# Aazmp/vp8oclenc

Measured on AMD Instinct MI355X. Metric: macroblocks/sec inter-frame (ME+DCT+loopfilter), 1080p, higher is better.
Workload: dtype u8/int32

## Files before the change

vp8oclenc_amd/csrc/kernels_mb.hip:

```cpp
#include <stdlib.h>
#include <string.h>

#include "vp8hip_dev.h"

namespace vp8 {


struct TDiv { uint32_t M8; bool one; };
struct Recip24 { uint32_t m8[512]; };
static constexpr Recip24 make_recip24() {
    Recip24 t{};
    for (uint32_t q = 0; q < 512; ++q) t.m8[q] = q < 2 ? 0u : (((1u << 24) / q + 1u) << 8);
    return t;
}
static __device__ __constant__ const Recip24 k_recip24 = make_recip24();
__device__ __forceinline__ TDiv tdiv_make(int q) { return TDiv{k_recip24.m8[q & 511], q == 1}; }
__device__ __forceinline__ int tdiv(int x, const TDiv &d) {
    const int s = x >> 31;
    const uint32_t n = (uint32_t)((x ^ s) - s);
    const uint32_t r = d.one ? n : __umulhi(n, d.M8);
    return ((int)r ^ s) - s;
}

constexpr uint32_t pk8t(int a, int b, int c, int d) {
    return (uint32_t)(a & 255) | ((uint32_t)(b & 255) << 8) | ((uint32_t)(c & 255) << 16) | ((uint32_t)(d & 255) << 24);
}
#define P6(f0, f1, f2, f3, f4, f5)                                                                          \
    {pk8t(f0, f1, f2, f3), pk8t(f4, f5, 0, 0), pk8t(0, f0, f1, f2), pk8t(f3, f4, f5, 0), pk8t(0, 0, f0, f1),  \
     pk8t(f2, f3, f4, f5), pk8t(0, 0, 0, f0),  pk8t(f1, f2, f3, f4), pk8t(f5, 0, 0, 0),  0, 0, 0}
static __device__ __constant__ const uint32_t K_P6[8][12] = {
    P6(0, 0, 0, 0, 0, 0),       P6(0, -6, 123, 12, -1, 0), P6(2, -11, 108, 36, -8, 1), P6(0, -9, 93, 50, -6, 0),
    P6(3, -16, 77, 77, -16, 3), P6(0, -6, 50, 93, -9, 0),  P6(1, -8, 36, 108, -11, 2), P6(0, -1, 12, 123, -6, 0)};
constexpr int KB6 = 128 * 128 + 64;
__device__ __forceinline__ int d4k(uint32_t a, uint32_t b, int c) { return __builtin_amdgcn_sdot4((int)a, (int)b, c, true); }
__device__ __forceinline__ int d4(uint32_t a, uint32_t b, int c) { return __builtin_amdgcn_sdot4((int)a, (int)b, c, false); }
__device__ __forceinline__ void six_tap4(uint32_t w0, uint32_t w1, uint32_t w2, const uint32_t t[9], int s[4]) {
    s[0] = d4(w1, t[1], d4k(w0, t[0], KB6));
    s[1] = d4(w1, t[3], d4k(w0, t[2], KB6));
    s[2] = d4(w1, t[5], d4k(w0, t[4], KB6));
    s[3] = d4(w2, t[8], d4(w1, t[7], d4k(w0, t[6], KB6)));
}
__device__ __forceinline__ uint32_t pack_sat4(const int s[4]) {
    const uint32_t lo = __builtin_amdgcn_ashr_pk_u8_i32(s[0], s[1], 7), hi = __builtin_amdgcn_ashr_pk_u8_i32(s[2], s[3], 7);
    return __builtin_amdgcn_perm(hi, lo, 0x05040100u);
}
template <bool CONFORMANT>
__device__ __forceinline__ void predict4x4(const Plane &rf, int ix, int iy, int fx, int fy, uint32_t out[4]) {
    uint32_t tx[9], ty[9];
#pragma unroll
    for (int i = 0; i < 9; ++i) { tx[i] = K_P6[fx][i]; ty[i] = K_P6[fy][i]; }
    uint32_t Hb[9];
#pragma unroll
    for (int L = 0; L < 9; ++L) {
        const uint8_t *p = rf.p + (ptrdiff_t)(iy - 2 + L) * rf.stride + (ix - 2);
        const uint32_t w0 = ld_u32(p) ^ 0x80808080u, w1 = ld_u32(p + 4) ^ 0x80808080u, w2 = ld_u32(p + 8) ^ 0x80808080u;
        int sm[4];
        six_tap4(w0, w1, w2, tx, sm);
        uint32_t h;
        if (L < 6 || CONFORMANT) {
            h = pack_sat4(sm);
        } else {
            h = 0;
#pragma unroll
            for (int c = 0; c < 4; ++c) h |= (uint32_t)(div128(sm[c]) & 0xff) << (8 * c);
        }
        h ^= 0x80808080u;
        Hb[L] = fx == 0 ? __builtin_amdgcn_alignbyte(w1, w0, 2) : h;
    }
    uint32_t ca[4], cb[4], oc[4];
    transpose4x4(Hb, ca);
    transpose4x4(Hb + 4, cb);
#pragma unroll
    for (int c = 0; c < 4; ++c) {
        int sm[4];
        six_tap4(ca[c], cb[c], Hb[8] >> (8 * c), ty, sm);
        const uint32_t v = pack_sat4(sm);
        oc[c] = fy == 0 ? (__builtin_amdgcn_alignbyte(cb[c], ca[c], 2) ^ 0x80808080u) : v;
    }
    transpose4x4(oc, out);
}

__device__ __forceinline__ void fdct4x4(const int in[16], int out[16]) {
    int L[16];
#pragma unroll
    for (int c = 0; c < 4; ++c) {
        const int r0 = in[c], r1 = in[4 + c], r2 = in[8 + c], r3 = in[12 + c];
        const int a1 = (r0 + r3) * 8, d1 = (r0 - r3) * 8, b1 = (r1 + r2) * 8, c1 = (r1 - r2) * 8;
        L[c] = a1 + b1;
        L[8 + c] = a1 - b1;
        const uint32_t xy = pk16(c1, d1);
        L[4 + c] = dot2(xy, K_ROT_A, 14500) >> 12;
        L[12 + c] = dot2(xy, K_ROT_B, 7500) >> 12;
    }
#pragma unroll
    for (int i = 0; i < 4; ++i) {
        const int e0 = L[4 * i], e1 = L[4 * i + 1], e2 = L[4 * i + 2], e3 = L[4 * i + 3];
        const int a1 = e0 + e3, d1 = e0 - e3, b1 = e1 + e2, c1 = e1 - e2;
        out[4 * i] = (a1 + b1 + 7) >> 4;
        out[4 * i + 2] = (a1 - b1 + 7) >> 4;
        const uint32_t xy = pk16(c1, d1);
        out[4 * i + 1] = (dot2(xy, K_ROT_A, 12000) >> 16) + (d1 != 0);
        out[4 * i + 3] = dot2(xy, K_ROT_B, 51000) >> 16;
    }
}

__device__ __forceinline__ void idct4x4(int L[16]) {
    int T[16];
#pragma unroll
    for (int c = 0; c < 4; ++c) {
        const int i0 = L[c], i1 = L[4 + c], i2 = L[8 + c], i3 = L[12 + c];
        const int a1 = i0 + i2, b1 = i0 - i2;
        const int c1 = (__mul24(i1, 35468) >> 16) - (i3 + (__mul24(i3, 20091) >> 16));
        const int d1 = (i1 + (__mul24(i1, 20091) >> 16)) + (__mul24(i3, 35468) >> 16);
        T[c] = a1 + d1;
        T[12 + c] = a1 - d1;
        T[4 + c] = b1 + c1;
        T[8 + c] = b1 - c1;
    }
#pragma unroll
    for (int r = 0; r < 4; ++r) {
        const int i0 = T[4 * r], i1 = T[4 * r + 1], i2 = T[4 * r + 2], i3 = T[4 * r + 3];
        const int a1 = i0 + i2, b1 = i0 - i2;
        const int c1 = (__mul24(i1, 35468) >> 16) - (i3 + (__mul24(i3, 20091) >> 16));
        const int d1 = (i1 + (__mul24(i1, 20091) >> 16)) + (__mul24(i3, 35468) >> 16);
        L[4 * r] = (a1 + d1 + 4) >> 3;
        L[4 * r + 3] = (a1 - d1 + 4) >> 3;
        L[4 * r + 1] = (b1 + c1 + 4) >> 3;
        L[4 * r + 2] = (b1 - c1 + 4) >> 3;
    }
}

__device__ __forceinline__ int had4(int v0, int v1, int v2, int v3, int i) {
    const int s1 = i >= 2 ? -1 : 1, s2 = (i == 1 || i == 2) ? -1 : 1, s3 = (i & 1) ? -1 : 1;
    return v0 + __mul24(s1, v1) + __mul24(s2, v2) + __mul24(s3, v3);
}
__device__ __forceinline__ int wht_roundtrip_lane(int x, int lane, int dc_q, int ac_q, const TDiv &ddc, const TDiv &dac, int &q) {
    const int L = lane & 15, r = L >> 2, c = L & 3;
    const int base = (int)(threadIdx.x & 32u) * 4;
    const int col = base + 4 * c, row = base + 4 * (L & 12);
    auto gather_col = [&](int v, int i) { return had4(__builtin_amdgcn_ds_bpermute(col, v), __builtin_amdgcn_ds_bpermute(col + 16, v),
                                                      __builtin_amdgcn_ds_bpermute(col + 32, v), __builtin_amdgcn_ds_bpermute(col + 48, v), i); };
    auto gather_row = [&](int v, int i) { return had4(__builtin_amdgcn_ds_bpermute(row, v), __builtin_amdgcn_ds_bpermute(row + 4, v),
                                                      __builtin_amdgcn_ds_bpermute(row + 8, v), __builtin_amdgcn_ds_bpermute(row + 12, v), i); };
    int o = gather_row(gather_col(x, r), c);
    o += (o > 0);
    o >>= 1;
    q = tdiv(o, L == 0 ? ddc : dac);
    const int xq = __mul24(q, L == 0 ? dc_q : ac_q);
    return (gather_col(gather_row(xq, c), r) + 3) >> 3;
}

__device__ __forceinline__ constexpr int inv_zigzag(int k) {
    constexpr int t[16] = {0, 1, 5, 6, 2, 4, 7, 12, 3, 8, 11, 13, 9, 10, 14, 15};
    return t[k];
}
__device__ __forceinline__ int inv_zigzag_rt(int k) { return (int)((0xfea9db83c7426510ull >> (4 * k)) & 15); }
__device__ __forceinline__ void store_zigzag(int16_t *dst, const int L[16]) {
    int z[16];
#pragma unroll
    for (int k = 0; k < 16; ++k) z[inv_zigzag(k)] = L[k];
    uint32_t w[8];
#pragma unroll
    for (int k = 0; k < 8; ++k) w[k] = (uint32_t)(uint16_t)z[2 * k] | ((uint32_t)(uint16_t)z[2 * k + 1] << 16);
    uint4 *d4 = reinterpret_cast<uint4 *>(dst);
    d4[0] = make_uint4(w[0], w[1], w[2], w[3]);
    d4[1] = make_uint4(w[4], w[5], w[6], w[7]);
}

struct MBPlanes { uint8_t *y, *u, *v; };
struct MBArgs {
    MBPlanes cur, ref0, ref1, ref2, recon;
    int ystride, cstride, yw, yh, cw, ch;
    int32_t *o_parts, *o_ref, *o_seg, *o_nz, *o_mask;
    int16_t *o_vec, *o_coeffs;
    float *o_ssim;
    int32_t *o_flag;
    const SegData *sd;
    const int32_t *bdiff0, *bdiff1, *bdiff2;
    const int16_t *vnet0, *vnet1, *vnet2;
    float ssim_target;
    int mbw, mbs;
    int use_golden, use_altref;
};

struct MBTile { uint8_t cur[384]; uint8_t rec[384]; float fa[384]; float fb[384]; };

__device__ __forceinline__ void tile_sums(const uint32_t *t32, int lane, int &sy, int &sc) {
    sy = (int)__builtin_amdgcn_sad_u8(t32[lane], 0u, __builtin_amdgcn_sad_u8(t32[lane + 32], 0u, 0u));
    sc = (int)__builtin_amdgcn_sad_u8(t32[64 + lane], 0u, 0u);
#pragma unroll
    for (int m = 16; m >= 1; m >>= 1) sy += __shfl_xor(sy, m, 32);
#pragma unroll
    for (int m = 8; m >= 1; m >>= 1) sc += __shfl_xor(sc, m, 32);
}
__device__ __forceinline__ float chain(const float *p, int n4) {
    float acc = 0.0f;
    for (int q = 0; q < n4; q += 4) {
        const float4 v = *reinterpret_cast<const float4 *>(p + q);
        acc = q == 0 ? v.x : __fadd_rn(v.x, acc);
        acc = __fadd_rn(v.y, acc);
        acc = __fadd_rn(v.z, acc);
        acc = __fadd_rn(v.w, acc);
    }
    return acc;
}
__device__ __forceinline__ float sum4(float acc, int lane) {
    const float s0 = __shfl(acc, (lane & ~3) + 0, 32), s1 = __shfl(acc, (lane & ~3) + 1, 32);
    const float s2 = __shfl(acc, (lane & ~3) + 2, 32), s3 = __shfl(acc, (lane & ~3) + 3, 32);
    return __fadd_rn(__fadd_rn(__fadd_rn(s0, s1), s2), s3);
}

template <bool CONFORMANT>
__device__ __forceinline__ void mb_body(const MBArgs &a, MBTile *s_t) {
    const int g = threadIdx.x >> 5, lane = threadIdx.x & 31;
    const int mb_raw = xcd_band(blockIdx.x, gridDim.x) * 8 + g;
    const bool live = mb_raw < a.mbs;
    const int mb = live ? mb_raw : a.mbs - 1;
    const int mbx = mb % a.mbw, mby = mb / a.mbw;
    const int32_t *SD = a.sd->v;

    const bool blk = lane < 24;
    const int plane = lane < 16 ? 0 : (lane < 20 ? 1 : 2);
    const int bi = lane < 16 ? lane : (lane - 16) & 3;
    const int bw = plane == 0 ? 4 : 2;
    const int bx = blk ? bi % bw : 0, by = blk ? bi / bw : 0;
    const int msz = plane == 0 ? 16 : 8;
    const int posx = mbx * msz + bx * 4, posy = mby * msz + by * 4;
    const int b8w = a.mbw * 2;
    const int cell0 = (mby * 2) * b8w + mbx * 2;
    const int cidx[4] = {cell0, cell0 + 1, cell0 + b8w, cell0 + b8w + 1};
    int diff1 = a.bdiff0[cidx[0]] + a.bdiff0[cidx[1]] + a.bdiff0[cidx[2]] + a.bdiff0[cidx[3]];
    int diff2 = 0x7fffffff;
    if (a.use_altref == 1)
        diff2 = a.bdiff2[cidx[0]] + a.bdiff2[cidx[1]] + a.bdiff2[cidx[2]] + a.bdiff2[cidx[3]];
    int ref = diff1 <= diff2 ? 0 : 2;
    diff1 = diff1 <= diff2 ? diff1 : diff2;
    diff2 = 0x7fffffff;
    if (a.use_golden == 1)
        diff2 = a.bdiff1[cidx[0]] + a.bdiff1[cidx[1]] + a.bdiff1[cidx[2]] + a.bdiff1[cidx[3]];
    ref = diff1 <= diff2 ? ref : 1;
    const uint32_t *vnet = reinterpret_cast<const uint32_t *>(ref == 0 ? a.vnet0 : (ref == 1 ? a.vnet1 : a.vnet2));
    uint32_t mbv[4];
#pragma unroll
    for (int k = 0; k < 4; ++k) mbv[k] = vnet[cidx[k]];
    const int parts = (mbv[1] == mbv[0] && mbv[2] == mbv[0] && mbv[3] == mbv[0]) ? 0 : 1;
    if (lane == 0 && live) {
        a.o_ref[mb] = ref;
        a.o_parts[mb] = parts;
        *reinterpret_cast<uint4 *>(a.o_vec + 8 * mb) = make_uint4(mbv[0], mbv[1], mbv[2], mbv[3]);
    }
    uint8_t *const rpy = ref == 0 ? a.ref0.y : (ref == 1 ? a.ref1.y : a.ref2.y);
    uint8_t *const rpu = ref == 0 ? a.ref0.u : (ref == 1 ? a.ref1.u : a.ref2.u);
    uint8_t *const rpv = ref == 0 ? a.ref0.v : (ref == 1 ? a.ref1.v : a.ref2.v);
    const int pstride = plane == 0 ? a.ystride : a.cstride, pw = plane == 0 ? a.yw : a.cw, ph = plane == 0 ? a.yh : a.ch;
    const Plane cp{plane == 0 ? a.cur.y : (plane == 1 ? a.cur.u : a.cur.v), pstride, pw, ph};
    const Plane rc{plane == 0 ? a.recon.y : (plane == 1 ? a.recon.u : a.recon.v), pstride, pw, ph};
    const Plane rp{plane == 0 ? rpy : (plane == 1 ? rpu : rpv), pstride, pw, ph};
    const int tile_off = plane == 0 ? 0 : (plane == 1 ? 256 : 320);

    uint32_t predw[4] = {0, 0, 0, 0};
    if (blk) {
        const int quad = plane == 0 ? (by >> 1) * 2 + (bx >> 1) : by * 2 + bx;
        const uint32_t vv = quad == 0 ? mbv[0] : (quad == 1 ? mbv[1] : (quad == 2 ? mbv[2] : mbv[3]));
        const int vx = (int16_t)(vv & 0xffffu), vy = (int16_t)(vv >> 16);
        const int gsh = plane == 0 ? 2 : 3, gm = plane == 0 ? 3 : 7;
        const int fxp = posx * (gm + 1) + vx, fyp = posy * (gm + 1) + vy;
        const int dx = (fxp & gm) * (plane == 0 ? 2 : 1), dy = (fyp & gm) * (plane == 0 ? 2 : 1);
        const int ix = iclamp(fxp >> gsh, 2 - EXT, rp.w + EXT - 7), iy = iclamp(fyp >> gsh, 2 - EXT, rp.h + EXT - 7);
        predict4x4<CONFORMANT>(rp, ix, iy, dx, dy, predw);
#pragma unroll
        for (int r = 0; r < 4; ++r) {
            const uint32_t cw = *reinterpret_cast<const uint32_t *>(cp.p + (ptrdiff_t)(posy + r) * cp.stride + posx);
            *reinterpret_cast<uint32_t *>(&s_t[g].cur[tile_off + (by * 4 + r) * msz + bx * 4]) = cw;
        }
    }
    const int sp = (lane >> 2) < 3 ? (lane >> 2) : 2, comp = lane & 3;
    const int n4 = sp == 0 ? 64 : 16;
    const int chain_off = (sp == 0 ? 0 : (sp == 1 ? 256 : 320)) + comp * n4;
    const float area = sp == 0 ? 256.0f : 64.0f;
    const uint32_t *cur32 = reinterpret_cast<const uint32_t *>(s_t[g].cur);
    const uint32_t *rec32 = reinterpret_cast<const uint32_t *>(s_t[g].rec);
    const int coff = (lane < 16 ? 256 : 320) + (lane & 15);
    float *fa = s_t[g].fa, *fb = s_t[g].fb;
    float M1y, M1c, M1, D1;
    {
        int sy, sc;
        tile_sums(cur32, lane, sy, sc);
        M1y = __fdiv_rn((float)sy, 256.0f);
        M1c = __fdiv_rn((float)sc, 64.0f);
        const float mu = __shfl(M1c, 0, 32), mv = __shfl(M1c, 16, 32);
        M1 = sp == 0 ? M1y : (sp == 1 ? mu : mv);
#pragma unroll
        for (int h = 0; h < 3; ++h) {
            const uint32_t w = cur32[h < 2 ? lane + 32 * h : 64 + lane];
            const float m = h < 2 ? M1y : M1c;
            const int off = h < 2 ? lane + 32 * h : coff, cs = h < 2 ? 64 : 16;
#pragma unroll
            for (int k = 0; k < 4; ++k) {
                const float t = __fsub_rn((float)byte_of(w, k), m);
                fa[off + k * cs] = __fmul_rn(t, t);
            }
        }
        D1 = __fdiv_rn(sum4(chain(fa + chain_off, n4), lane), area);
    }

    float ssim = -2.0f;
    int seg_final = a.o_seg[mb];
    int nz_blk = 0;
    bool any_pass = false;

    for (int seg = 3; seg >= 0; --seg) {
        if (ssim > a.ssim_target) break;
        {
        any_pass = true;
        seg_final = seg;
        const int i = SD[seg * SD_INTS + SD_Y_AC_I];
        int dc_q, ac_q;
        if (plane == 0) {
            ac_q = k_ac_q[i];
            dc_q = parts == 0 ? 1 : k_dc_q[qi(SD[SD_Y_DC_IDELTA] + i)];
        } else {
            dc_q = imin(k_dc_q[qi(SD[SD_UV_DC_IDELTA] + i)], 132);
            ac_q = k_ac_q[qi(SD[SD_UV_AC_IDELTA] + i)];
        }
        int coef[16];
#pragma unroll
        for (int k = 0; k < 16; ++k) coef[k] = 0;
        if (blk) {
            int res[16];
#pragma unroll
            for (int r = 0; r < 4; ++r) {
                const uint32_t cw = *reinterpret_cast<const uint32_t *>(&s_t[g].cur[tile_off + (by * 4 + r) * msz + bx * 4]);
#pragma unroll
                for (int c = 0; c < 4; ++c) res[4 * r + c] = byte_of(cw, c) - byte_of(predw[r], c);
            }
            fdct4x4(res, coef);
            const TDiv ddc = tdiv_make(dc_q), dac = tdiv_make(ac_q);
            coef[0] = tdiv(coef[0], ddc);
#pragma unroll
            for (int k = 1; k < 16; ++k) coef[k] = tdiv(coef[k], dac);
        }
        nz_blk = 0;
        if (parts == 0) {
            const int y2dc = k_dc_q[qi(SD[SD_Y2_DC_IDELTA] + i)] * 2;
            const int y2ac = imax(31 * k_ac_q[qi(SD[SD_Y2_AC_IDELTA] + i)] / 20, 8);
            int q24 = 0;
            const int nd = wht_roundtrip_lane((int16_t)coef[0], lane, y2dc, y2ac, tdiv_make(y2dc), tdiv_make(y2ac), q24);
            if (lane < 16) {
                coef[0] = (int16_t)nd;
                if (live) a.o_coeffs[((size_t)mb * 25 + 24) * 16 + inv_zigzag_rt(lane)] = (int16_t)q24;
                nz_blk += iabs((int16_t)q24);
            }
        }
        if (blk) {
            if (live) store_zigzag(a.o_coeffs + ((size_t)mb * 25 + lane) * 16, coef);
#pragma unroll
            for (int k = 1; k < 16; ++k) nz_blk += iabs((int16_t)coef[k]);
            if (plane != 0 || parts != 0) nz_blk += iabs((int16_t)coef[0]);
            int L[16];
            L[0] = __mul24((int16_t)coef[0], dc_q);
#pragma unroll
            for (int k = 1; k < 16; ++k) L[k] = __mul24((int16_t)coef[k], ac_q);
            idct4x4(L);
#pragma unroll
            for (int r = 0; r < 4; ++r) {
                uint32_t w = 0;
#pragma unroll
                for (int c = 0; c < 4; ++c) w |= (uint32_t)sat8(L[4 * r + c] + byte_of(predw[r], c)) << (8 * c);
                *reinterpret_cast<uint32_t *>(&s_t[g].rec[tile_off + (by * 4 + r) * msz + bx * 4]) = w;
                if (live) *reinterpret_cast<uint32_t *>(rc.p + (ptrdiff_t)(posy + r) * rc.stride + posx) = w;
            }
        }
        }
        {
        float M2, D, C;
        {
            int sy, sc;
            tile_sums(rec32, lane, sy, sc);
            const float M2y = __fdiv_rn((float)sy, 256.0f), M2c = __fdiv_rn((float)sc, 64.0f);
            const float mu = __shfl(M2c, 0, 32), mv = __shfl(M2c, 16, 32);
            M2 = sp == 0 ? M2y : (sp == 1 ? mu : mv);
#pragma unroll
            for (int h = 0; h < 3; ++h) {
                const int di = h < 2 ? lane + 32 * h : 64 + lane;
                const uint32_t wc = cur32[di], wr = rec32[di];
                const float m1 = h < 2 ? M1y : M1c, m2 = h < 2 ? M2y : M2c;
                const int off = h < 2 ? lane + 32 * h : coff, cs = h < 2 ? 64 : 16;
#pragma unroll
                for (int k = 0; k < 4; ++k) {
                    const float t1 = __fsub_rn((float)byte_of(wc, k), m1);
                    const float t2 = __fsub_rn((float)byte_of(wr, k), m2);
                    fa[off + k * cs] = __fmul_rn(t2, t2);
                    fb[off + k * cs] = __fmul_rn(t1, t2);
                }
            }
            D = __fadd_rn(D1, __fdiv_rn(sum4(chain(fa + chain_off, n4), lane), area));
            C = __fdiv_rn(sum4(chain(fb + chain_off, n4), lane), area);
        }
        const float k1 = 0.01f * 0.01f * 255 * 255, k2 = 0.03f * 0.03f * 255 * 255;
        const float num = __fmul_rn(__fadd_rn(__fmul_rn(M1, __fmul_rn(M2, 2.0f)), k1), __fadd_rn(__fmul_rn(C, 2.0f), k2));
        const float den = __fmul_rn(__fadd_rn(__fmul_rn(M1, M1), __fadd_rn(__fmul_rn(M2, M2), k1)), __fadd_rn(D, k2));
        float metric = __fdiv_rn(num, den);
        float dm = __fsub_rn(M1, M2);
        dm = dm < 0 ? -dm : dm;
        dm = dm > 4 ? __fmul_rn(0.02f, dm) : 0.0f;
        metric = __fsub_rn(metric, dm);
        const float m1 = __shfl(metric, 0, 32), m2 = __shfl(metric, 4, 32), m3 = __shfl(metric, 8, 32);
        ssim = __fdiv_rn(__fadd_rn(__fadd_rn(m1, m2), m3), 3.0f);
        }
    }

    int nz = any_pass ? nz_blk : 0;
#pragma unroll
    for (int m = 16; m >= 1; m >>= 1) nz += __shfl_xor(nz, m, 32);
    if (lane == 0 && live) {
        if (any_pass) {
            a.o_seg[mb] = seg_final;
            a.o_nz[mb] = nz;
            a.o_mask[mb] = (parts != 0 || nz > 0) ? -1 : 0;
        }
        a.o_ssim[mb] = ssim;
        if (ssim < a.ssim_target) *a.o_flag = 1;
    }
}

struct MBShare {
    float M1[8][4], M2[8][4], D1[8][4], metric[8][4];
    int nzc[8];
    int any[2];
};
struct MBTileP { MBTile t; uint32_t skew[4]; };
template <int CTRL>
__device__ __forceinline__ int dpp_i(int v) { return __builtin_amdgcn_update_dpp(0, v, CTRL, 0xf, 0xf, false); }
template <int CTRL>
__device__ __forceinline__ float dpp_f(float v) { return __builtin_bit_cast(float, dpp_i<CTRL>(__builtin_bit_cast(int, v))); }
__device__ __forceinline__ int quad_sum(int v) {
    v += dpp_i<0xb1>(v);
    return v + dpp_i<0x4e>(v);
}
__device__ __forceinline__ int half_row_sum(int v) { v = quad_sum(v); return v + dpp_i<0x141>(v); }
__device__ __forceinline__ int row_sum(int v) { v = half_row_sum(v); return v + dpp_i<0x140>(v); }
__device__ __forceinline__ float sum4_quad(float acc) {
    return __fadd_rn(__fadd_rn(__fadd_rn(dpp_f<0x00>(acc), dpp_f<0x55>(acc)), dpp_f<0xaa>(acc)), dpp_f<0xff>(acc));
}
template <int N4>
__device__ __forceinline__ float chain_n(const float *p) {
    float acc = 0.0f;
#pragma unroll 4
    for (int q = 0; q < N4; q += 4) {
        const float4 v = *reinterpret_cast<const float4 *>(p + q);
        acc = q == 0 ? v.x : __fadd_rn(v.x, acc);
        acc = __fadd_rn(v.y, acc);
        acc = __fadd_rn(v.z, acc);
        acc = __fadd_rn(v.w, acc);
    }
    return acc;
}
__device__ __forceinline__ int wht_roundtrip_row(int x, int L, int base_bytes, int dc_q, int ac_q, const TDiv &ddc, const TDiv &dac, int &q) {
    const int r = L >> 2, c = L & 3;
    const int col = base_bytes + 4 * c, row = base_bytes + 4 * (L & 12);
    auto gather_col = [&](int v, int i) { return had4(__builtin_amdgcn_ds_bpermute(col, v), __builtin_amdgcn_ds_bpermute(col + 16, v),
                                                      __builtin_amdgcn_ds_bpermute(col + 32, v), __builtin_amdgcn_ds_bpermute(col + 48, v), i); };
    auto gather_row = [&](int v, int i) { return had4(__builtin_amdgcn_ds_bpermute(row, v), __builtin_amdgcn_ds_bpermute(row + 4, v),
                                                      __builtin_amdgcn_ds_bpermute(row + 8, v), __builtin_amdgcn_ds_bpermute(row + 12, v), i); };
    int o = gather_row(gather_col(x, r), c);
    o += (o > 0);
    o >>= 1;
    q = tdiv(o, L == 0 ? ddc : dac);
    const int xq = __mul24(q, L == 0 ? dc_q : ac_q);
    return (gather_col(gather_row(xq, c), r) + 3) >> 3;
}

template <bool CONFORMANT>
__device__ __forceinline__ void mb_body_packed(const MBArgs &a, MBTileP *s_t, MBShare *s_x) {
    const int w = __builtin_amdgcn_readfirstlane((int)(threadIdx.x >> 6)), wl = threadIdx.x & 63;
    const bool luma = w < 2;
    const int g = luma ? w * 4 + (wl >> 4) : wl >> 3;
    const int plane = luma ? 0 : 1 + ((wl >> 2) & 1);
    const int bi = luma ? wl & 15 : wl & 3;
    const int blkidx = luma ? bi : 12 + 4 * plane + bi;
    const int mb_raw = xcd_band(blockIdx.x, gridDim.x) * 8 + g;
    const bool live = mb_raw < a.mbs;
    const int mb = live ? mb_raw : a.mbs - 1;
    const int mbx = mb % a.mbw, mby = mb / a.mbw;
    const int32_t *SD = a.sd->v;
    const int bw = luma ? 4 : 2;
    const int bx = bi % bw, by = bi / bw;
    const int msz = luma ? 16 : 8;
    const int posx = mbx * msz + bx * 4, posy = mby * msz + by * 4;
    if (threadIdx.x == 0) s_x->any[0] = s_x->any[1] = 0;
    const int b8w = a.mbw * 2;
    const int cell0 = (mby * 2) * b8w + mbx * 2;
    const int cidx[4] = {cell0, cell0 + 1, cell0 + b8w, cell0 + b8w + 1};
    int diff1 = a.bdiff0[cidx[0]] + a.bdiff0[cidx[1]] + a.bdiff0[cidx[2]] + a.bdiff0[cidx[3]];
    int diff2 = 0x7fffffff;
    if (a.use_altref == 1)
        diff2 = a.bdiff2[cidx[0]] + a.bdiff2[cidx[1]] + a.bdiff2[cidx[2]] + a.bdiff2[cidx[3]];
    int ref = diff1 <= diff2 ? 0 : 2;
    diff1 = diff1 <= diff2 ? diff1 : diff2;
    diff2 = 0x7fffffff;
    if (a.use_golden == 1)
        diff2 = a.bdiff1[cidx[0]] + a.bdiff1[cidx[1]] + a.bdiff1[cidx[2]] + a.bdiff1[cidx[3]];
    ref = diff1 <= diff2 ? ref : 1;
    const uint32_t *vnet = reinterpret_cast<const uint32_t *>(ref == 0 ? a.vnet0 : (ref == 1 ? a.vnet1 : a.vnet2));
    uint32_t mbv[4];
#pragma unroll
    for (int k = 0; k < 4; ++k) mbv[k] = vnet[cidx[k]];
    const int parts = (mbv[1] == mbv[0] && mbv[2] == mbv[0] && mbv[3] == mbv[0]) ? 0 : 1;
    const bool head = luma && bi == 0;
    if (head && live) {
        a.o_ref[mb] = ref;
        a.o_parts[mb] = parts;
        *reinterpret_cast<uint4 *>(a.o_vec + 8 * mb) = make_uint4(mbv[0], mbv[1], mbv[2], mbv[3]);
    }
    uint8_t *const rpy = ref == 0 ? a.ref0.y : (ref == 1 ? a.ref1.y : a.ref2.y);
    uint8_t *const rpu = ref == 0 ? a.ref0.u : (ref == 1 ? a.ref1.u : a.ref2.u);
    uint8_t *const rpv = ref == 0 ? a.ref0.v : (ref == 1 ? a.ref1.v : a.ref2.v);
    const int pstride = luma ? a.ystride : a.cstride, pw = luma ? a.yw : a.cw, ph = luma ? a.yh : a.ch;
    const Plane cp{plane == 0 ? a.cur.y : (plane == 1 ? a.cur.u : a.cur.v), pstride, pw, ph};
    const Plane rc{plane == 0 ? a.recon.y : (plane == 1 ? a.recon.u : a.recon.v), pstride, pw, ph};
    const Plane rp{plane == 0 ? rpy : (plane == 1 ? rpu : rpv), pstride, pw, ph};
    const int tile_off = plane == 0 ? 0 : (plane == 1 ? 256 : 320);
    MBTile &T = s_t[g].t;

    uint32_t predw[4];
    {
        const int quad = luma ? (by >> 1) * 2 + (bx >> 1) : by * 2 + bx;
        const uint32_t vv = quad == 0 ? mbv[0] : (quad == 1 ? mbv[1] : (quad == 2 ? mbv[2] : mbv[3]));
        const int vx = (int16_t)(vv & 0xffffu), vy = (int16_t)(vv >> 16);
        const int gsh = luma ? 2 : 3, gm = luma ? 3 : 7;
        const int fxp = posx * (gm + 1) + vx, fyp = posy * (gm + 1) + vy;
        const int dx = (fxp & gm) * (luma ? 2 : 1), dy = (fyp & gm) * (luma ? 2 : 1);
        const int ix = iclamp(fxp >> gsh, 2 - EXT, rp.w + EXT - 7), iy = iclamp(fyp >> gsh, 2 - EXT, rp.h + EXT - 7);
        predict4x4<CONFORMANT>(rp, ix, iy, dx, dy, predw);
#pragma unroll
        for (int r = 0; r < 4; ++r) {
            const uint32_t cw = *reinterpret_cast<const uint32_t *>(cp.p + (ptrdiff_t)(posy + r) * cp.stride + posx);
            *reinterpret_cast<uint32_t *>(&T.cur[tile_off + (by * 4 + r) * msz + bx * 4]) = cw;
        }
    }
    const uint32_t *cur32 = reinterpret_cast<const uint32_t *>(T.cur) + (tile_off >> 2);
    const uint32_t *rec32 = reinterpret_cast<const uint32_t *>(T.rec) + (tile_off >> 2);
    const int dstep = luma ? 16 : 4, cs = luma ? 64 : 16;
    const float area = luma ? 256.0f : 64.0f;
    float *fa = T.fa + tile_off + bi, *fb = T.fb + tile_off + bi;
    auto plane_sum = [&](const uint32_t *t32) {
        uint32_t s = 0;
#pragma unroll
        for (int h = 0; h < 4; ++h) s = __builtin_amdgcn_sad_u8(t32[bi + dstep * h], 0u, s);
        return luma ? row_sum((int)s) : quad_sum((int)s);
    };
    const float M1 = __fdiv_rn((float)plane_sum(cur32), area);
#pragma unroll
    for (int h = 0; h < 4; ++h) {
        const uint32_t wd = cur32[bi + dstep * h];
#pragma unroll
        for (int k = 0; k < 4; ++k) {
            const float t = __fsub_rn((float)byte_of(wd, k), M1);
            fa[dstep * h + k * cs] = __fmul_rn(t, t);
        }
    }
    if (bi == 0) s_x->M1[g][plane] = M1;
    __syncthreads();
    if (w == 0) {
        if (wl < 32) {
            const int m = wl >> 2, comp = wl & 3;
            const float s = sum4_quad(chain_n<64>(s_t[m].t.fa + comp * 64));
            if (comp == 0) s_x->D1[m][0] = __fdiv_rn(s, 256.0f);
        }
    } else if (w == 1) {
        const int m = wl >> 3, p = 1 + ((wl >> 2) & 1), comp = wl & 3;
        const float s = sum4_quad(chain_n<16>(s_t[m].t.fa + (p == 1 ? 256 : 320) + comp * 16));
        if (comp == 0) s_x->D1[m][p] = __fdiv_rn(s, 64.0f);
    }
    __syncthreads();

    float ssim = -2.0f;
    int seg_final = a.o_seg[mb];
    int nz_y = 0, nz_c = 0;
    bool any_pass = false;
    for (int seg = 3, round = 0; seg >= 0; --seg, ++round) {
        const bool act = !(ssim > a.ssim_target);
        if (act) {
            any_pass = true;
            seg_final = seg;
            const int i = SD[seg * SD_INTS + SD_Y_AC_I];
            int dc_q, ac_q;
            if (luma) {
                ac_q = k_ac_q[i];
                dc_q = parts == 0 ? 1 : k_dc_q[qi(SD[SD_Y_DC_IDELTA] + i)];
            } else {
                dc_q = imin(k_dc_q[qi(SD[SD_UV_DC_IDELTA] + i)], 132);
                ac_q = k_ac_q[qi(SD[SD_UV_AC_IDELTA] + i)];
            }
            int coef[16];
            {
                int res[16];
#pragma unroll
                for (int r = 0; r < 4; ++r) {
                    const uint32_t cw = *reinterpret_cast<const uint32_t *>(&T.cur[tile_off + (by * 4 + r) * msz + bx * 4]);
#pragma unroll
                    for (int c = 0; c < 4; ++c) res[4 * r + c] = byte_of(cw, c) - byte_of(predw[r], c);
                }
                fdct4x4(res, coef);
                const TDiv ddc = tdiv_make(dc_q), dac = tdiv_make(ac_q);
                coef[0] = tdiv(coef[0], ddc);
#pragma unroll
                for (int k = 1; k < 16; ++k) coef[k] = tdiv(coef[k], dac);
            }
            int nz_blk = 0;
            if (luma && parts == 0) {
                const int y2dc = k_dc_q[qi(SD[SD_Y2_DC_IDELTA] + i)] * 2;
                const int y2ac = imax(31 * k_ac_q[qi(SD[SD_Y2_AC_IDELTA] + i)] / 20, 8);
                int q24 = 0;
                const int nd = wht_roundtrip_row((int16_t)coef[0], bi, (wl & 48) * 4, y2dc, y2ac, tdiv_make(y2dc), tdiv_make(y2ac), q24);
                coef[0] = (int16_t)nd;
                if (live) a.o_coeffs[((size_t)mb * 25 + 24) * 16 + inv_zigzag_rt(bi)] = (int16_t)q24;
                nz_blk += iabs((int16_t)q24);
            }
            {
                if (live) store_zigzag(a.o_coeffs + ((size_t)mb * 25 + blkidx) * 16, coef);
#pragma unroll
                for (int k = 1; k < 16; ++k) nz_blk += iabs((int16_t)coef[k]);
                if (!luma || parts != 0) nz_blk += iabs((int16_t)coef[0]);
                int L[16];
                L[0] = __mul24((int16_t)coef[0], dc_q);
#pragma unroll
                for (int k = 1; k < 16; ++k) L[k] = __mul24((int16_t)coef[k], ac_q);
                idct4x4(L);
#pragma unroll
                for (int r = 0; r < 4; ++r) {
                    uint32_t wd = 0;
#pragma unroll
                    for (int c = 0; c < 4; ++c) wd |= (uint32_t)sat8(L[4 * r + c] + byte_of(predw[r], c)) << (8 * c);
                    *reinterpret_cast<uint32_t *>(&T.rec[tile_off + (by * 4 + r) * msz + bx * 4]) = wd;
                    if (live) *reinterpret_cast<uint32_t *>(rc.p + (ptrdiff_t)(posy + r) * rc.stride + posx) = wd;
                }
            }
            if (luma) nz_y = row_sum(nz_blk);
            else {
                const int n = half_row_sum(nz_blk);
                if ((wl & 7) == 0) s_x->nzc[g] = n;
            }
            const float M2 = __fdiv_rn((float)plane_sum(rec32), area);
#pragma unroll
            for (int h = 0; h < 4; ++h) {
                const uint32_t wc = cur32[bi + dstep * h], wr = rec32[bi + dstep * h];
#pragma unroll
                for (int k = 0; k < 4; ++k) {
                    const float t1 = __fsub_rn((float)byte_of(wc, k), M1);
                    const float t2 = __fsub_rn((float)byte_of(wr, k), M2);
                    fa[dstep * h + k * cs] = __fmul_rn(t2, t2);
                    fb[dstep * h + k * cs] = __fmul_rn(t1, t2);
                }
            }
            if (bi == 0) {
                s_x->M2[g][plane] = M2;
                s_x->any[round & 1] = 1;
            }
        }
        __syncthreads();
        if (!s_x->any[round & 1]) break;
        if (threadIdx.x == 0) s_x->any[(round + 1) & 1] = 0;
        {
            const int comp = wl & 3;
            const int m = w == 0 ? (wl >> 2) & 7 : (w - 1) * 4 + ((wl >> 3) & 3);
            const int p = w == 0 ? 0 : 1 + ((wl >> 2) & 1);
            const float *src = (wl < 32 ? s_t[m].t.fa : s_t[m].t.fb) + (p == 0 ? 0 : (p == 1 ? 256 : 320)) + comp * (w == 0 ? 64 : 16);
            const float acc = w == 0 ? chain_n<64>(src) : chain_n<16>(src);
            const float s = __fdiv_rn(sum4_quad(acc), w == 0 ? 256.0f : 64.0f);
            const float C = __shfl_xor(s, 32, 64);
            const float D = __fadd_rn(s_x->D1[m][p], s);
            const float m1v = s_x->M1[m][p], m2v = s_x->M2[m][p];
            const float k1 = 0.01f * 0.01f * 255 * 255, k2 = 0.03f * 0.03f * 255 * 255;
            const float num = __fmul_rn(__fadd_rn(__fmul_rn(m1v, __fmul_rn(m2v, 2.0f)), k1), __fadd_rn(__fmul_rn(C, 2.0f), k2));
            const float den = __fmul_rn(__fadd_rn(__fmul_rn(m1v, m1v), __fadd_rn(__fmul_rn(m2v, m2v), k1)), __fadd_rn(D, k2));
            float metric = __fdiv_rn(num, den);
            float dm = __fsub_rn(m1v, m2v);
            dm = dm < 0 ? -dm : dm;
            dm = dm > 4 ? __fmul_rn(0.02f, dm) : 0.0f;
            metric = __fsub_rn(metric, dm);
            if (wl < 32 && comp == 0) s_x->metric[m][p] = metric;
        }
        if (act && luma) nz_c = s_x->nzc[g];
        __syncthreads();
        const float4 mt = *reinterpret_cast<const float4 *>(s_x->metric[g]);
        ssim = __fdiv_rn(__fadd_rn(__fadd_rn(mt.x, mt.y), mt.z), 3.0f);
    }

    if (head && live) {
        if (any_pass) {
            const int nz = nz_y + nz_c;
            a.o_seg[mb] = seg_final;
            a.o_nz[mb] = nz;
            a.o_mask[mb] = (parts != 0 || nz > 0) ? -1 : 0;
        }
        a.o_ssim[mb] = ssim;
        if (ssim < a.ssim_target) *a.o_flag = 1;
    }
}

__global__ __launch_bounds__(256, 2) void k_mb_b(BatchOf<MBArgs> b) {
    __shared__ __attribute__((aligned(16))) MBTile s_t[8];
    mb_body<false>(b.item[blockIdx.z], s_t);
}
__global__ __launch_bounds__(256, 2) void k_mb_b_conformant(BatchOf<MBArgs> b) {
    __shared__ __attribute__((aligned(16))) MBTile s_t[8];
    mb_body<true>(b.item[blockIdx.z], s_t);
}

__global__ __launch_bounds__(192, 2) void k_mb_p(BatchOf<MBArgs> b) {
    __shared__ __attribute__((aligned(16))) MBTileP s_t[8];
    __shared__ __attribute__((aligned(16))) MBShare s_x;
    mb_body_packed<false>(b.item[blockIdx.z], s_t, &s_x);
}
__global__ __launch_bounds__(192, 2) void k_mb_p_conformant(BatchOf<MBArgs> b) {
    __shared__ __attribute__((aligned(16))) MBTileP s_t[8];
    __shared__ __attribute__((aligned(16))) MBShare s_x;
    mb_body_packed<true>(b.item[blockIdx.z], s_t, &s_x);
}
static bool mb_packed() {
    static const bool on = [] { const char *v = getenv("VP8HIP_MB_PACKED"); return !(v && v[0] == '0'); }();
    return on;
}

static MBArgs mb_args(const CodingItem &it, float ssim_target, int mbw, int mbh) {
    const Frame &cur = *it.cur, &recon = *it.recon;
    const RefSet &refs = it.refs;
    const NetSet &nets = *it.nets;
    const MBOut &o = *it.out;
    MBArgs a;
    auto planes = [](const Frame &f) { return MBPlanes{f.Y[0].p, f.U.p, f.V.p}; };
    a.cur = planes(cur);
    a.ref0 = planes(refs.ref[0]); a.ref1 = planes(refs.ref[1]); a.ref2 = planes(refs.ref[2]);
    a.recon = planes(recon);
    a.ystride = cur.Y[0].stride; a.yw = cur.Y[0].w; a.yh = cur.Y[0].h;
    a.cstride = cur.U.stride; a.cw = cur.U.w; a.ch = cur.U.h;
    a.o_parts = o.parts; a.o_ref = o.ref; a.o_seg = o.seg; a.o_nz = o.nz; a.o_mask = o.mask;
    a.o_vec = o.vec; a.o_coeffs = o.coeffs; a.o_ssim = o.ssim; a.o_flag = o.flags;
    a.sd = it.sd;
    a.bdiff0 = nets.bdiff[0]; a.bdiff1 = nets.bdiff[1]; a.bdiff2 = nets.bdiff[2];
    a.vnet0 = nets.net[0][0]; a.vnet1 = nets.net[1][0]; a.vnet2 = nets.net[2][0];
    a.ssim_target = ssim_target;
    a.mbw = mbw;
    a.mbs = mbw * mbh;
    a.use_golden = refs.use[1];
    a.use_altref = refs.use[2];
    return a;
}
static bool mb_skip() {
    static const bool skip = experiment_skip("mb");
    return skip;
}

void launch_mb_batch(hipStream_t s, const CodingItem *items, int n, float ssim_target, int mbw, int mbh, bool conformant) {
    static_assert(sizeof(BatchOf<MBArgs>) <= 4096, "the batch travels in the kernel arguments");
    BatchOf<MBArgs> b;
    b.n = n;
    for (int i = 0; i < n; ++i) b.item[i] = mb_args(items[i], ssim_target, mbw, mbh);
    if (mb_skip()) return;
    const dim3 grid((b.item[0].mbs + 7) / 8, 1, n);
    if (mb_packed()) {
        if (conformant) VP8_LAUNCH(k_mb_p_conformant, grid, dim3(192), 0, s, b);
        else VP8_LAUNCH(k_mb_p, grid, dim3(192), 0, s, b);
        return;
    }
    if (conformant) VP8_LAUNCH(k_mb_b_conformant, grid, dim3(256), 0, s, b);
    else VP8_LAUNCH(k_mb_b, grid, dim3(256), 0, s, b);
}

__global__ __launch_bounds__(256) void k_filter_mask(MBOut o, const SegData *sd, int mbs) {
    const int lane = threadIdx.x & 31;
    const int mb_raw = blockIdx.x * 8 + (threadIdx.x >> 5);
    const bool live = mb_raw < mbs;
    const int mb = live ? mb_raw : mbs - 1;
    const int parts = o.parts[mb];
    int nz = 0;
    if (lane < 25) {
        const int16_t *c = o.coeffs + ((size_t)mb * 25 + lane) * 16;
        int s = 0;
#pragma unroll
        for (int k = 1; k < 16; ++k) s += iabs(c[k]);
        if (lane < 16) nz = s + (parts != 0 ? iabs(c[0]) : 0);
        else if (lane < 24) nz = s + iabs(c[0]);
        else nz = parts == 0 ? s + iabs(c[0]) : 0;
    }
#pragma unroll
    for (int m = 16; m >= 1; m >>= 1) nz += __shfl_xor(nz, m, 32);
    if (lane == 0 && live) {
        o.nz[mb] = nz;
        o.mask[mb] = (parts != 0 || nz > 0) ? -1 : 0;
    }
}

void launch_filter_mask(hipStream_t s, const MBOut &o, const SegData *d_sd, int mbs) {
    hipLaunchKernelGGL(k_filter_mask, dim3((mbs + 7) / 8), dim3(256), 0, s, o, d_sd, mbs);
}

}
```

vp8oclenc_amd/csrc/kernels_me.hip:

```cpp
#include <stdlib.h>
#include <string.h>

#include "vp8hip_dev.h"
#include "s1_pre_layout.h"
#include "s1_fill_layout.h"

namespace vp8 {

struct BorderItem { Plane y, u, v; };
static_assert(EXT == 8, "border_row stores a margin as one eight-byte word");
__device__ __forceinline__ void border_row(const Plane &pl, int row, int lane) {
    if (row >= pl.h + EXT) return;
    uint8_t *dst = pl.p + (ptrdiff_t)row * pl.stride;
    const uint8_t *src = pl.p + (ptrdiff_t)iclamp(row, 0, pl.h - 1) * pl.stride;
    if (row < 0 || row >= pl.h)
        for (int x = lane * 8; x < pl.w; x += 512) *reinterpret_cast<uint2 *>(dst + x) = *reinterpret_cast<const uint2 *>(src + x);
    if (lane < 2) {
        const uint32_t s4 = (uint32_t)src[lane ? pl.w - 1 : 0] * 0x01010101u;
        *reinterpret_cast<uint2 *>(dst + (lane ? pl.w : -EXT)) = make_uint2(s4, s4);
    }
}
__device__ __forceinline__ void border_body(const BorderItem &a) {
    border_row(blockIdx.y == 0 ? a.y : (blockIdx.y == 1 ? a.u : a.v), (int)blockIdx.x - EXT, threadIdx.x);
}

__global__ __launch_bounds__(64) void k_border(BorderItem a) { border_body(a); }

void launch_border(hipStream_t s, const Frame &f) {
    dim3 grid(f.Y[0].h + 2 * EXT, 3);
    VP8_LAUNCH(k_border, grid, dim3(64), 0, s, BorderItem{f.Y[0], f.U, f.V});
}

struct PyrArgs { Frame f[2 * MAX_BATCH]; uint32_t border_mask; };
static int border_jobs(const Frame &f) { return (f.Y[0].h + 2 * EXT) + 2 * (f.U.h + 2 * EXT); }

__global__ __launch_bounds__(256) void k_pyramid(PyrArgs a) {
    __shared__ uint8_t s2[16][16];
    __shared__ uint8_t s3[8][8];
    const Frame &f = a.f[blockIdx.z];
    const int t = threadIdx.x, tx = t & 15, ty = t >> 4;
    const Plane &P0 = f.Y[0];
    const int tiles_y = (P0.h + 63) / 64;
    const int tile = xcd_band((int)blockIdx.y * (int)gridDim.x + (int)blockIdx.x, tiles_y * (int)gridDim.x);
    const int bx = tile % (int)gridDim.x, by = tile / (int)gridDim.x;
    if ((int)blockIdx.y >= tiles_y) {
        if (!((a.border_mask >> blockIdx.z) & 1)) return;
        int job = (((int)blockIdx.y - tiles_y) * (int)gridDim.x + (int)blockIdx.x) * 4 + (t >> 6);
        const int ny = P0.h + 2 * EXT, nc = f.U.h + 2 * EXT;
        if (job < ny) border_row(P0, job - EXT, t & 63);
        else if (job < ny + nc) border_row(f.U, job - ny - EXT, t & 63);
        else if (job < ny + 2 * nc) border_row(f.V, job - ny - nc - EXT, t & 63);
        return;
    }
    const int sx = imin(bx * 64 + 4 * tx, P0.w - 4), sy0 = by * 64 + 4 * ty;
    uint32_t r[4];
#pragma unroll
    for (int k = 0; k < 4; ++k)
        r[k] = *reinterpret_cast<const uint32_t *>(P0.p + (ptrdiff_t)imin(sy0 + k, P0.h - 1) * P0.stride + sx);
    int l1[2][2];
#pragma unroll
    for (int j = 0; j < 2; ++j)
#pragma unroll
        for (int i = 0; i < 2; ++i)
            l1[j][i] = (byte_of(r[2 * j], 2 * i) + byte_of(r[2 * j], 2 * i + 1) + byte_of(r[2 * j + 1], 2 * i) +
                        byte_of(r[2 * j + 1], 2 * i + 1) + 2) >> 2;
    const Plane &P1 = f.Y[1];
    const int x1 = bx * 32 + 2 * tx, y1 = by * 32 + 2 * ty;
    if (x1 < P1.w) {
#pragma unroll
        for (int j = 0; j < 2; ++j)
            if (y1 + j < P1.h)
                *reinterpret_cast<uint16_t *>(P1.p + (ptrdiff_t)(y1 + j) * P1.stride + x1) = (uint16_t)(l1[j][0] | (l1[j][1] << 8));
    }
    const int l2 = (l1[0][0] + l1[0][1] + l1[1][0] + l1[1][1] + 2) >> 2;
    const Plane &P2 = f.Y[2];
    const int x2 = bx * 16 + tx, y2 = by * 16 + ty;
    if (x2 < P2.w && y2 < P2.h) P2.p[(ptrdiff_t)y2 * P2.stride + x2] = (uint8_t)l2;
    s2[ty][tx] = (uint8_t)l2;
    __syncthreads();
    if (t < 64) {
        const int ux = t & 7, uy = t >> 3;
        const int l3 = (s2[2 * uy][2 * ux] + s2[2 * uy][2 * ux + 1] + s2[2 * uy + 1][2 * ux] + s2[2 * uy + 1][2 * ux + 1] + 2) >> 2;
        const Plane &P3 = f.Y[3];
        const int x3 = bx * 8 + ux, y3 = by * 8 + uy;
        if (x3 < P3.w && y3 < P3.h) P3.p[(ptrdiff_t)y3 * P3.stride + x3] = (uint8_t)l3;
        s3[uy][ux] = (uint8_t)l3;
    }
    __syncthreads();
    if (t < 16) {
        const int ux = t & 3, uy = t >> 2;
        const int l4 = (s3[2 * uy][2 * ux] + s3[2 * uy][2 * ux + 1] + s3[2 * uy + 1][2 * ux] + s3[2 * uy + 1][2 * ux + 1] + 2) >> 2;
        const Plane &P4 = f.Y[4];
        const int x4 = bx * 4 + ux, y4 = by * 4 + uy;
        if (x4 < P4.w && y4 < P4.h) P4.p[(ptrdiff_t)y4 * P4.stride + x4] = (uint8_t)l4;
    }
}

static dim3 pyramid_grid(const Frame &f, int nframes, uint32_t border_mask) {
    const int gx = (f.Y[0].w + 63) / 64, gy = (f.Y[0].h + 63) / 64;
    const int extra = border_mask ? ((border_jobs(f) + 3) / 4 + gx - 1) / gx : 0;
    return dim3(gx, gy + extra, nframes);
}
void launch_pyramid(hipStream_t s, const Frame *a, const Frame *b, uint32_t border_mask) {
    PyrArgs p;
    p.f[0] = *a;
    p.f[1] = b ? *b : *a;
    p.border_mask = border_mask;
    VP8_LAUNCH(k_pyramid, pyramid_grid(*a, b ? 2 : 1, border_mask), dim3(256), 0, s, p);
}
void launch_pyramid_batch(hipStream_t s, const Frame *const *f, int nframes, uint32_t border_mask) {
    if (nframes <= 0) return;
    PyrArgs p;
    for (int i = 0; i < nframes; ++i) p.f[i] = *f[i];
    p.border_mask = border_mask;
    VP8_LAUNCH(k_pyramid, pyramid_grid(*f[0], nframes, border_mask), dim3(256), 0, s, p);
}

struct PackItem { Plane py, pu, pv; const uint8_t *sy, *su, *sv; int sw, sh, ssy, ssc; };
__device__ __forceinline__ void pack_body(const PackItem &a, int per) {
    const Plane &py = a.py, &pu = a.pu, &pv = a.pv;
    const uint8_t *sy = a.sy, *su = a.su, *sv = a.sv;
    const int ny = (py.w >> 3) * py.h, nc = (pu.w >> 3) * pu.h;
    for (int k = 0; k < per; ++k) {
        int i = ((int)blockIdx.x * per + k) * 256 + (int)threadIdx.x;
        const Plane *pl = &py;
        const uint8_t *src = sy;
        int sw = a.sw, sh = a.sh, ss = a.ssy;
        if (i >= ny) {
            i -= ny;
            pl = &pu;
            src = su;
            sw >>= 1; sh >>= 1; ss = a.ssc;
            if (i >= nc) { i -= nc; pl = &pv; src = sv; }
            if (i >= nc) return;
        }
        const int upr = pl->w >> 3;
        const int y = i / upr, x = (i % upr) * 8;
        const uint8_t *row = src + (size_t)(y < sh ? y : sh - 1) * ss;
        uint2 v;
        if (x + 8 <= sw && ((ss | (int)(reinterpret_cast<uintptr_t>(src) & 7)) & 7) == 0) {
            v = *reinterpret_cast<const uint2 *>(row + x);
        } else {
            uint32_t w[2] = {0, 0};
#pragma unroll
            for (int j = 0; j < 8; ++j) w[j >> 2] |= (uint32_t)row[x + j < sw ? x + j : sw - 1] << (8 * (j & 3));
            v = make_uint2(w[0], w[1]);
        }
        *reinterpret_cast<uint2 *>(pl->p + (ptrdiff_t)y * pl->stride + x) = v;
    }
}

__global__ __launch_bounds__(256) void k_pack_b(BatchOf<PackItem> b, int per) { pack_body(b.item[blockIdx.z], per); }
static int pack_units_per_thread() {
    static const int per = [] { const char *e = getenv("VP8HIP_PACK_UNITS"); const int v = e ? atoi(e) : 16; return v < 1 ? 1 : (v > 64 ? 64 : v); }();
    return per;
}

static PackItem pack_item(const Frame &f, const void *y, const void *u, const void *v, int sw, int sh, int ssy, int ssc) {
    if (sw <= 0) { sw = f.Y[0].w; sh = f.Y[0].h; }
    if (ssy <= 0) { ssy = sw; ssc = sw >> 1; }
    return PackItem{f.Y[0], f.U, f.V, (const uint8_t *)y, (const uint8_t *)u, (const uint8_t *)v, sw, sh, ssy, ssc};
}
void launch_pack_batch(hipStream_t s, const SourceItem *items, int n, int sw, int sh, int ssy, int ssc) {
    BatchOf<PackItem> b;
    b.n = n;
    for (int i = 0; i < n; ++i) b.item[i] = pack_item(*items[i].f, items[i].y, items[i].u, items[i].v, sw, sh, ssy, ssc);
    const Frame &f = *items[0].f;
    const int units = (f.Y[0].w >> 3) * f.Y[0].h + 2 * ((f.U.w >> 3) * f.U.h);
    const int per = pack_units_per_thread();
    VP8_LAUNCH(k_pack_b, dim3((units + 256 * per - 1) / (256 * per), 1, n), dim3(256), 0, s, b, per);
}

struct Search1Args {
    Plane cur;
    Plane ref[3];
    const int16_t *src[3];
    int16_t *dst[3];
    int refmap[3];
    int nrefs;
    int net_width, w, h, pixel_rate, rate_shift, nblk, bw;
    int pbw, pbh;
    uint32_t bw_inv;
};

template <bool SPLIT>
struct S1Map {
    static constexpr int LANES_PER_BLOCK = SPLIT ? 20 : 5;
    static constexpr int BLOCKS_PER_WAVE = SPLIT ? 3 : 12;
    static constexpr int BLOCKS_PER_WG = 4 * BLOCKS_PER_WAVE;
};

__device__ __forceinline__ void s1_subblock(const uint8_t *cp, int cstride, const uint8_t *rp, int rstride, int acc[5]) {
    uint32_t c[4], q0[4], q1[4];
#pragma unroll
    for (int y = 0; y < 4; ++y) {
        c[y] = *reinterpret_cast<const uint32_t *>(cp + (ptrdiff_t)y * cstride) ^ 0x80808080u;
        const uint2 q = ld_u64(rp + (ptrdiff_t)y * rstride);
        q0[y] = q.x ^ 0x80808080u; q1[y] = q.y ^ 0x80808080u;
    }
    uint32_t cc[4], col[8];
    transpose4x4(c, cc);
    transpose4x4(q0, col);
    transpose4x4(q1, col + 4);
    int pre[16];
#pragma unroll
    for (int k = 0; k < 4; ++k) weight_pre_column(cc[k], pre + 4 * k);
#pragma unroll
    for (int i = 0; i < 5; ++i) acc[i] += weight_cols_pre(pre, col + i);
}

__device__ __forceinline__ void s1_subblock_pre(v4i wa, const int *pre_lds, int pre_off, const uint8_t *rp, int rstride, int acc[5]) {
    uint32_t q0[4], q1[4];
#pragma unroll
    for (int y = 0; y < 4; ++y) {
        q0[y] = ld_u32(rp + (ptrdiff_t)y * rstride) ^ 0x80808080u;
        q1[y] = ld_u32(rp + (ptrdiff_t)y * rstride + 4) ^ 0x80808080u;
    }
#pragma unroll
    for (int i = 0; i < 5; ++i) {
        int off = pre_off;
        asm volatile("" : "+v"(off));
        __builtin_amdgcn_sched_barrier(0);
        v4i b;
#pragma unroll
        for (int y = 0; y < 4; ++y) b[y] = i == 0 ? (int)q0[y] : i == 4 ? (int)q1[y] : (int)__builtin_amdgcn_alignbyte(q1[y], q0[y], (uint32_t)i);
        acc[i] += weight_mfma(wa, load_pre16(pre_lds + off), b);
    }
}
static_assert(s1_pre_c_read_worst() == 4 && s1_pre_c_read_best() == 4, "the C reads of the whole-pel search's pre table must be free of LDS bank conflicts");
static_assert(S1_PRE_BLOCKS == S1Map<false>::BLOCKS_PER_WAVE, "s1_pre_layout.h and the loop form's lane map disagree");
__device__ __forceinline__ void s1_make_pre(const Plane &cur, int cx, int cy, int sb, bool on, int *dst16) {
    const int sx = (sb >> 1) * 4, sy = (sb & 1) * 4;
    const uint8_t *cp = cur.p + (ptrdiff_t)(cy + sy) * cur.stride + cx + sx;
    uint32_t c[4], cc[4];
#pragma unroll
    for (int y = 0; y < 4; ++y) c[y] = *reinterpret_cast<const uint32_t *>(cp + (ptrdiff_t)y * cur.stride) ^ 0x80808080u;
    transpose4x4(c, cc);
    int pre[16];
    weight_pre_block(cc, pre);
    if (on) {
#pragma unroll
        for (int k = 0; k < 4; ++k) *reinterpret_cast<int4 *>(dst16 + 4 * k) = make_int4(pre[4 * k], pre[4 * k + 1], pre[4 * k + 2], pre[4 * k + 3]);
    }
}

template <bool SPLIT, bool PRE_LDS = false, bool LDS_MIN = false>
__device__ __forceinline__ uint32_t search1_block(const Search1Args &a, int r, int cx, int cy, uint32_t pv, bool live, int sub, int lane,
                                                  const int *pre_lds = nullptr ,
                                                  int pre_off = 0 ,
                                                  uint32_t *min_lds = nullptr ) {
    const int sb0 = sub / 5, j = sub - 5 * sb0;
    int v0x = (int16_t)(pv & 0xffffu), v0y = (int16_t)(pv >> 16);
    const int rmask = a.pixel_rate - 1;
    v0x = (v0x + ((v0x >> 31) & rmask)) >> a.rate_shift;
    v0y = (v0y + ((v0y >> 31) & rmask)) >> a.rate_shift;
    if (a.pixel_rate > 8) v0x = v0y = 0;

    const int py = (int16_t)(cy + v0y + (j - 2));
    const bool row_valid = live && py >= 0 && py <= a.h - 8;
    const int xb = cx + v0x - 2;
    const bool loadable = row_valid && xb >= -8 && xb <= a.w - 4;
    const int lx = loadable ? xb : cx, ly = loadable ? py : cy;

    const uint8_t *cp = a.cur.p + (ptrdiff_t)cy * a.cur.stride + cx;
    const uint8_t *rp = a.ref[r].p + (ptrdiff_t)ly * a.ref[r].stride + lx;
    int acc[5] = {0, 0, 0, 0, 0};
    if (SPLIT) {
        const int sx = (sb0 >> 1) * 4, sy = (sb0 & 1) * 4;
        s1_subblock(cp + (ptrdiff_t)sy * a.cur.stride + sx, a.cur.stride, rp + (ptrdiff_t)sy * a.ref[r].stride + sx, a.ref[r].stride, acc);
#pragma unroll
        for (int i = 0; i < 5; ++i) {
            acc[i] += __shfl(acc[i], lane + 10, 64);
            acc[i] += __shfl(acc[i], lane + 5, 64);
        }
    } else {
        if (PRE_LDS) {
            const v4i wa = metric_a_rows(lane);
#pragma unroll 1
            for (int sb = 0; sb < 4; ++sb) {
                const int sx = (sb >> 1) * 4, sy = (sb & 1) * 4;
                s1_subblock_pre(wa, pre_lds, pre_off + s1_pre_sub_at(sb), rp + (ptrdiff_t)sy * a.ref[r].stride + sx, a.ref[r].stride, acc);
            }
        } else {
#pragma unroll 1
            for (int sb = 0; sb < 4; ++sb) {
                const int sx = (sb >> 1) * 4, sy = (sb & 1) * 4;
                s1_subblock(cp + (ptrdiff_t)sy * a.cur.stride + sx, a.cur.stride, rp + (ptrdiff_t)sy * a.ref[r].stride + sx, a.ref[r].stride, acc);
            }
        }
    }
    const int pen_mask = a.pixel_rate < 4 ? -1 : 0;
    const int pen_y = iabs(iabs(py - cy) - v0y);
    uint32_t best = 0xffffffffu;
#pragma unroll
    for (int i = 0; i < 5; ++i) {
        const int px = (int16_t)(xb + i);
        const bool valid = loadable && px >= 0 && px <= a.w - 8;
        const int diff = (acc[i] + (((iabs(iabs(px - cx) - v0x) + pen_y) << 5) & pen_mask)) & 0xffff;
        const uint32_t key = (valid && diff < 0x7fff) ? ((uint32_t)diff << 8) | (uint32_t)(j * 5 + i) : 0xffffffffu;
        best = key < best ? key : best;
    }
    if (LDS_MIN) {
        min_lds[sub] = best;
        __syncthreads();
#pragma unroll
        for (int k = 0; k < 5; ++k) {
            const uint32_t o = min_lds[k];
            best = o < best ? o : best;
        }
    } else {
#pragma unroll
        for (int off = 1; off <= 4; off <<= 1) {
            const uint32_t o = (uint32_t)__shfl((int)best, lane + off, 64);
            if (j + off < 5 && o < best) best = o;
        }
    }
    int bx, by;
    if (best != 0xffffffffu) {
        const int k = best & 0xff;
        bx = v0x + (k % 5 - 2);
        by = v0y + (k / 5 - 2);
    } else {
        bx = (int16_t)(v0x - cx);
        by = (int16_t)(v0y - cy);
    }
    const uint32_t ox16 = (uint16_t)(int16_t)((int16_t)bx * (int16_t)a.pixel_rate);
    const uint32_t oy16 = (uint16_t)(int16_t)((int16_t)by * (int16_t)a.pixel_rate);
    return ox16 | (oy16 << 16);
}

static_assert(s1_fill_c_read_worst() == 4 && s1_fill_c_read_best() == 4, "the C reads of the filled loop form's pre table must be free of LDS bank conflicts: all four waves, every sub-block and quad");
static_assert(s1_fill_c_read_worst(64) > 4, "the bank model sees the conflicts of unskewed slots");
template <bool SPLIT, bool PRE_LDS = false, bool REF_LOOP = false, bool FILL = false>
__device__ __forceinline__ void search1_body(const Search1Args &a) {
    using M = S1Map<SPLIT>;
    static_assert(!FILL || (!SPLIT && PRE_LDS && REF_LOOP), "the filled map is the loop form's, with the table in LDS and the reference loop");
    if (!REF_LOOP && (int)blockIdx.y >= a.nrefs) return;
    const int lane = threadIdx.x & 63, wave = threadIdx.x >> 6;
    const int grp = FILL ? s1_fill_slot_of((int)threadIdx.x) : lane / M::LANES_PER_BLOCK;
    const int sub = FILL ? (int)threadIdx.x - S1_FILL_LANES * grp : lane - M::LANES_PER_BLOCK * grp;
    const int b_raw = FILL ? s1_fill_block_of(xcd_band(blockIdx.x, gridDim.x), grp, a.nblk) : (xcd_band(blockIdx.x, gridDim.x) * 4 + wave) * M::BLOCKS_PER_WAVE + grp;
    const bool live = FILL ? b_raw >= 0 : grp < M::BLOCKS_PER_WAVE && b_raw < a.nblk;
    const int b = live ? b_raw : a.nblk - 1;
    const int by = a.bw == 1 ? b : (int)__umulhi((uint32_t)b, a.bw_inv), bx = b - by * a.bw;
    const int cx = bx * 8, cy = by * 8;
    const int parent = (cy >> 4) * a.net_width + (cx >> 4);
    const bool parent_written = (cx >> 4) < a.pbw && (cy >> 4) < a.pbh;
    const int *pre_lds = nullptr;
    int pre_off = 0;
    uint32_t *min_lds = nullptr;
    if (FILL) {
        __shared__ __attribute__((aligned(16))) int s_fill[S1_FILL_INTS];
        __shared__ uint32_t s_min[2][S1_FILL_MIN_WORDS];
        const int t = threadIdx.x, slot = s1_fill_task_slot(t), sb = s1_fill_task_sub(t);
        const int tb_raw = xcd_band(blockIdx.x, gridDim.x) * S1_FILL_BLOCKS + slot;
        const int tb = tb_raw < a.nblk ? tb_raw : a.nblk - 1;
        const int tby = a.bw == 1 ? tb : (int)__umulhi((uint32_t)tb, a.bw_inv), tbx = tb - tby * a.bw;
        s1_make_pre(a.cur, tbx * 8, tby * 8, sb, slot < S1_FILL_BLOCKS, s_fill + s1_fill_slot_at(slot) + s1_pre_sub_at(sb));
        __syncthreads();
        pre_lds = s_fill;
        pre_off = s1_fill_c_at(t, 0, 0);
        min_lds = &s_min[0][s1_fill_min_at(t)];
    } else if (!SPLIT && PRE_LDS) {
        __shared__ __attribute__((aligned(16))) int s_pre[4][S1_PRE_INTS];
        const int slot = lane >> 2, sb = lane & 3;
        const int tb_raw = (xcd_band(blockIdx.x, gridDim.x) * 4 + wave) * M::BLOCKS_PER_WAVE + slot;
        const int tb = tb_raw < a.nblk ? tb_raw : a.nblk - 1;
        const int tby = a.bw == 1 ? tb : (int)__umulhi((uint32_t)tb, a.bw_inv), tbx = tb - tby * a.bw;
        s1_make_pre(a.cur, tbx * 8, tby * 8, sb, slot < M::BLOCKS_PER_WAVE, &s_pre[0][0] + s1_pre_slot_at(wave, slot) + s1_pre_sub_at(sb));
        asm volatile("s_waitcnt lgkmcnt(0)" ::: "memory");
        pre_lds = &s_pre[0][0];
        pre_off = s1_pre_c_at(wave, lane, 0, 0);
    }
    const int nr = REF_LOOP ? a.nrefs : 1;
#pragma unroll 1
    for (int ri = 0; ri < nr; ++ri) {
        const int r = a.refmap[REF_LOOP ? ri : (int)blockIdx.y];
        const uint32_t pv = parent_written ? reinterpret_cast<const uint32_t *>(a.src[r])[parent] : 0u;
        const uint32_t out = search1_block<SPLIT, !SPLIT && PRE_LDS, FILL>(a, r, cx, cy, pv, live, sub, lane, pre_lds, pre_off,
                                                                            FILL ? min_lds + (ri & 1) * S1_FILL_MIN_WORDS : nullptr);
        if (sub == 0 && live) {
            const int cell = (cy >> 3) * a.net_width + (cx >> 3);
            reinterpret_cast<uint32_t *>(a.dst[r])[cell] = out;
        }
    }
}

struct CoarseArgs { Search1Args lv[5]; };
constexpr int COARSE_WAVES = 6;
template <bool FINEST, bool TOP_ONLY = false>
__device__ __forceinline__ void coarse_tile(const Search1Args &L0, const Search1Args &L1, const Search1Args &L2, const Search1Args &L3, const Search1Args &L4, int r) {
    using M = S1Map<true>;
    __shared__ uint32_t mv4, mv3, mv2[4], mv1[16];
    const int lane = threadIdx.x & 63, wave = threadIdx.x >> 6;
    const int grp = lane / M::LANES_PER_BLOCK, sub = lane - M::LANES_PER_BLOCK * grp;
    const int slot = grp < M::BLOCKS_PER_WAVE ? wave * M::BLOCKS_PER_WAVE + grp : 99;
    const int tiles_x = (L1.bw + 3) / 4;
    const int tile = xcd_band(blockIdx.x, gridDim.x);
    const int ty = tile / tiles_x, tx = tile - ty * tiles_x;
    {
        const int bx = tx >> 1, by = ty >> 1;
        const bool exists = bx < L4.bw && by * L4.bw + bx < L4.nblk;
        if (wave == 0) {
            const bool live = slot == 0 && exists;
            const uint32_t out = search1_block<true>(L4, r, (live ? bx : 0) * 8, (live ? by : 0) * 8, 0u, live, sub, lane);
            if (slot == 0 && sub == 0) mv4 = exists ? out : 0u;
        }
    }
    __syncthreads();
    {
        const bool exists = tx < L3.bw && ty * L3.bw + tx < L3.nblk;
        if (wave == 0) {
            const bool live = slot == 0 && exists;
            const uint32_t out = search1_block<true>(L3, r, (live ? tx : 0) * 8, (live ? ty : 0) * 8, mv4, live, sub, lane);
            if (slot == 0 && sub == 0) mv3 = exists ? out : 0u;
        }
    }
    __syncthreads();
    if (wave < 2) {
        const int i = slot & 1, j = (slot >> 1) & 1;
        const int bx = 2 * tx + i, by = 2 * ty + j;
        const bool exists = slot < 4 && bx < L2.bw && by * L2.bw + bx < L2.nblk;
        const uint32_t out = search1_block<true>(L2, r, (exists ? bx : 0) * 8, (exists ? by : 0) * 8, mv3, exists, sub, lane);
        if (slot < 4 && sub == 0) mv2[slot] = exists ? out : 0u;
        if (TOP_ONLY && slot < 4 && sub == 0 && exists) reinterpret_cast<uint32_t *>(L2.dst[r])[by * L2.net_width + bx] = out;
    }
    if (TOP_ONLY) return;
    __syncthreads();
    {
        const int i = slot & 3, j = (slot >> 2) & 3;
        const int bx = 4 * tx + i, by = 4 * ty + j;
        const bool live = slot < 16 && bx < L1.bw && by * L1.bw + bx < L1.nblk;
        const uint32_t pv = mv2[(((j >> 1) & 1) << 1) | ((i >> 1) & 1)];
        const uint32_t out = search1_block<true>(L1, r, (live ? bx : 0) * 8, (live ? by : 0) * 8, pv, live, sub, lane);
        if (sub == 0 && live) reinterpret_cast<uint32_t *>(L1.dst[r])[by * L1.net_width + bx] = out;
        if (FINEST && sub == 0 && slot < 16) mv1[slot] = live ? out : 0u;
    }
    if (!FINEST) return;
    __syncthreads();
    {
        using M0 = S1Map<false>;
        const int grp0 = lane / M0::LANES_PER_BLOCK, sub0 = lane - M0::LANES_PER_BLOCK * grp0;
        const int slot0 = grp0 < M0::BLOCKS_PER_WAVE ? wave * M0::BLOCKS_PER_WAVE + grp0 : 99;
        const int i = slot0 & 7, j = (slot0 >> 3) & 7;
        const int bx = 8 * tx + i, by = 8 * ty + j;
        const bool live = slot0 < 64 && bx < L0.bw && by * L0.bw + bx < L0.nblk;
        const uint32_t pv = mv1[((j >> 1) << 2) | (i >> 1)];
        const uint32_t out = search1_block<false>(L0, r, (live ? bx : 0) * 8, (live ? by : 0) * 8, pv, live, sub0, lane);
        if (sub0 == 0 && live) reinterpret_cast<uint32_t *>(L0.dst[r])[by * L0.net_width + bx] = out;
    }
}

template <bool FINEST>
__global__ __launch_bounds__(64 * COARSE_WAVES) void k_search1_coarse(CoarseArgs a) {
    if ((int)blockIdx.y >= a.lv[1].nrefs) return;
    coarse_tile<FINEST>(a.lv[0], a.lv[1], a.lv[2], a.lv[3], a.lv[4], a.lv[1].refmap[blockIdx.y]);
}

struct CoarseGeom { int w, h, cur_stride, ref_stride; };
struct CoarseMember {
    const uint8_t *cur[5];
    const uint8_t *ref[3][5];
    int16_t *dst1[3], *dst0[3];
    int refmap[3], nrefs;
};
struct CoarseBatchArgs { CoarseGeom g[5]; int net_width, n; CoarseMember m[MAX_BATCH]; };
static_assert(sizeof(CoarseBatchArgs) <= 4096, "a batch's argument block travels in the 4 KiB kernel-argument segment");
__device__ __forceinline__ Search1Args coarse_level(const CoarseBatchArgs &a, const CoarseMember &m, int l, int r) {
    Search1Args s;
    const CoarseGeom &g = a.g[l];
    s.cur = Plane{const_cast<uint8_t *>(m.cur[l]), g.cur_stride, g.w, g.h};
    s.ref[0] = Plane{const_cast<uint8_t *>(m.ref[r][l]), g.ref_stride, g.w, g.h};
    s.dst[0] = l == 1 ? m.dst1[r] : m.dst0[r];
    s.net_width = a.net_width;
    s.w = g.w;
    s.h = g.h;
    s.pixel_rate = 1 << l;
    s.rate_shift = l;
    s.bw = g.w / 8;
    s.nblk = (g.w / 8) * (g.h / 8);
    return s;
}
__global__ __launch_bounds__(128) void k_search1_top_b(CoarseBatchArgs a) {
    const CoarseMember &m = a.m[blockIdx.z];
    if ((int)blockIdx.y >= m.nrefs) return;
    const int r = m.refmap[blockIdx.y];
    const Search1Args L1 = coarse_level(a, m, 1, r), L2 = coarse_level(a, m, 2, r), L3 = coarse_level(a, m, 3, r), L4 = coarse_level(a, m, 4, r);
    coarse_tile<false, true>(L1, L1, L2, L3, L4, 0);
}
template <bool FINEST>
__global__ __launch_bounds__(64 * COARSE_WAVES) void k_search1_coarse_b(CoarseBatchArgs a) {
    const CoarseMember &m = a.m[blockIdx.z];
    if ((int)blockIdx.y >= m.nrefs) return;
    const int r = m.refmap[blockIdx.y];
    const Search1Args L0 = coarse_level(a, m, 0, r), L1 = coarse_level(a, m, 1, r), L2 = coarse_level(a, m, 2, r), L3 = coarse_level(a, m, 3, r),
                      L4 = coarse_level(a, m, 4, r);
    coarse_tile<FINEST>(L0, L1, L2, L3, L4, 0);
}

template <bool SPLIT>
__global__ __launch_bounds__(256) void k_search1(Search1Args a) { search1_body<SPLIT>(a); }
static_assert(sizeof(BatchOf<Search1Args>) <= 4096 && sizeof(PyrArgs) <= 4096 && sizeof(BatchOf<PackItem>) <= 4096, "a batch's argument blocks travel in the 4 KiB kernel-argument segment");
template <bool SPLIT>
__global__ __launch_bounds__(256) void k_search1_b(BatchOf<Search1Args> b) { search1_body<SPLIT>(b.item[blockIdx.z]); }
__global__ __attribute__((amdgpu_waves_per_eu(8, 8))) __launch_bounds__(256) void k_search1_pl(Search1Args a) { search1_body<false, true>(a); }
__global__ __attribute__((amdgpu_waves_per_eu(8, 8))) __launch_bounds__(256) void k_search1_pl_b(BatchOf<Search1Args> b) { search1_body<false, true>(b.item[blockIdx.z]); }
__global__ __attribute__((amdgpu_waves_per_eu(7, 8))) __launch_bounds__(256) void k_search1_plr_b(BatchOf<Search1Args> b) { search1_body<false, true, true, true>(b.item[blockIdx.z]); }
static bool search1_ref_loop() {
    static const bool on = [] { const char *v = getenv("VP8HIP_S1_REF_LOOP"); return !(v && v[0] == '0'); }();
    return on;
}
static bool search1_pre_lds() {
    static const bool on = [] { const char *v = getenv("VP8HIP_S1_PRE_LDS"); return !(v && v[0] == '0'); }();
    return on;
}

static Search1Args search1_args(const CodingItem &it, int level, int src_idx, int net_width) {
    const Frame &cur = *it.cur;
    const RefSet &refs = it.refs;
    const NetSet &nets = *it.nets;
    Search1Args a;
    a.cur = cur.Y[level];
    int n = 0;
    for (int r = 0; r < 3; ++r) {
        a.ref[r] = refs.ref[r].Y[level];
        a.src[r] = nets.net[r][src_idx];
        a.dst[r] = nets.net[r][src_idx ^ 1];
        if (refs.use[r]) a.refmap[n++] = r;
    }
    a.nrefs = n;
    for (int i = n; i < 3; ++i) a.refmap[i] = 0;
    a.net_width = net_width;
    a.w = a.cur.w;
    a.h = a.cur.h;
    a.pixel_rate = 1 << level;
    a.rate_shift = level;
    a.bw = a.w / 8;
    a.nblk = (a.w / 8) * (a.h / 8);
    a.bw_inv = a.bw > 0 ? (uint32_t)(((1ull << 32) + a.bw - 1) / a.bw) : 0;
    a.pbw = level < 4 ? cur.Y[level + 1].w / 8 : 0;
    a.pbh = level < 4 ? cur.Y[level + 1].h / 8 : 0;
    return a;
}

int persistent_workgroups() {
    static const int n = [] { const char *v = getenv("VP8HIP_PERSIST"); return v && v[0] ? atoi(v) : 0; }();
    return n;
}

static bool search1_skip() {
    static const bool skip = experiment_skip("s1");
    return skip;
}
static bool search1_split(size_t blocks_times_refs, bool latency) {
    static const int forced = [] { const char *v = getenv("VP8HIP_S1_SPLIT"); return v && v[0] ? (v[0] == '1' ? 1 : 0) : -1; }();
    return forced >= 0 ? forced == 1 : (latency || blocks_times_refs < (size_t)12 * 1024);
}

void launch_search1(hipStream_t s, const CodingItem &it, int level, int src_idx, int net_width, bool latency) {
    const Search1Args a = search1_args(it, level, src_idx, net_width);
    const int n = a.nrefs;
    if (a.nblk <= 0 || n == 0 || search1_skip()) return;
    if (search1_split((size_t)a.nblk * n, latency))
        VP8_LAUNCH(k_search1<true>, dim3((a.nblk + S1Map<true>::BLOCKS_PER_WG - 1) / S1Map<true>::BLOCKS_PER_WG, n), dim3(256), 0, s, a);
    else if (search1_pre_lds())
        VP8_LAUNCH(k_search1_pl, dim3((a.nblk + S1Map<false>::BLOCKS_PER_WG - 1) / S1Map<false>::BLOCKS_PER_WG, n), dim3(256), 0, s, a);
    else
        VP8_LAUNCH(k_search1<false>, dim3((a.nblk + S1Map<false>::BLOCKS_PER_WG - 1) / S1Map<false>::BLOCKS_PER_WG, n), dim3(256), 0, s, a);
}

void launch_search1_coarse(hipStream_t s, const CodingItem &it, int net_width, bool finest) {
    CoarseArgs a;
    for (int l = 0; l <= 4; ++l) a.lv[l] = search1_args(it, l, l & 1, net_width);
    const Search1Args &L0 = a.lv[0], &L1 = a.lv[1];
    if (L0.nblk <= 0 || L0.nrefs == 0 || search1_skip()) return;
    const int tiles_x = finest ? (L0.bw + 7) / 8 : (L1.bw + 3) / 4, tiles_y = finest ? (L0.h / 8 + 7) / 8 : (L1.h / 8 + 3) / 4;
    if (tiles_x * tiles_y <= 0) return;
    if (finest) VP8_LAUNCH(k_search1_coarse<true>, dim3(tiles_x * tiles_y, L0.nrefs), dim3(64 * COARSE_WAVES), 0, s, a);
    else VP8_LAUNCH(k_search1_coarse<false>, dim3(tiles_x * tiles_y, L0.nrefs), dim3(64 * COARSE_WAVES), 0, s, a);
}

bool launch_search1_coarse_batch(hipStream_t s, const CodingItem *items, int n, int net_width, bool finest, bool top_only) {
    CoarseBatchArgs a;
    a.net_width = net_width;
    a.n = n;
    int maxrefs = 0;
    for (int l = 0; l <= 4; ++l) {
        const Plane &c = items[0].cur->Y[l];
        a.g[l] = CoarseGeom{c.w, c.h, c.stride, items[0].refs.ref[0].Y[l].stride};
    }
    for (int i = 0; i < n; ++i) {
        CoarseMember &m = a.m[i];
        const RefSet &refs = items[i].refs;
        const NetSet &nets = *items[i].nets;
        int k = 0;
        for (int r = 0; r < 3; ++r) {
            for (int l = 0; l <= 4; ++l) {
                const Plane &rp = refs.ref[r].Y[l], &cp = items[i].cur->Y[l];
                if (rp.stride != a.g[l].ref_stride || cp.stride != a.g[l].cur_stride || cp.w != a.g[l].w || cp.h != a.g[l].h || rp.w != cp.w || rp.h != cp.h) return false;
                m.ref[r][l] = rp.p;
                if (r == 0) m.cur[l] = cp.p;
            }
            m.dst1[r] = nets.net[r][0];
            m.dst0[r] = nets.net[r][1];
            if (refs.use[r]) m.refmap[k++] = r;
        }
        m.nrefs = k;
        for (int j = k; j < 3; ++j) m.refmap[j] = 0;
        maxrefs = k > maxrefs ? k : maxrefs;
    }
    const int bw0 = a.g[0].w / 8, bh0 = a.g[0].h / 8, bw1 = a.g[1].w / 8, bh1 = a.g[1].h / 8;
    if (bw0 * bh0 <= 0 || maxrefs == 0 || search1_skip()) return true;
    const int tiles_x = finest ? (bw0 + 7) / 8 : (bw1 + 3) / 4, tiles_y = finest ? (bh0 + 7) / 8 : (bh1 + 3) / 4;
    if (tiles_x * tiles_y <= 0) return !finest ? true : false;
    if (top_only) {
        VP8_LAUNCH(k_search1_top_b, dim3(tiles_x * tiles_y, maxrefs, n), dim3(128), 0, s, a);
        return true;
    }
    if (finest) VP8_LAUNCH(k_search1_coarse_b<true>, dim3(tiles_x * tiles_y, maxrefs, n), dim3(64 * COARSE_WAVES), 0, s, a);
    else VP8_LAUNCH(k_search1_coarse_b<false>, dim3(tiles_x * tiles_y, maxrefs, n), dim3(64 * COARSE_WAVES), 0, s, a);
    return true;
}

void launch_search1_batch(hipStream_t s, const CodingItem *items, int n, int level, int src_idx, int net_width) {
    BatchOf<Search1Args> b;
    b.n = n;
    int maxrefs = 0, totrefs = 0;
    for (int i = 0; i < n; ++i) {
        b.item[i] = search1_args(items[i], level, src_idx, net_width);
        maxrefs = b.item[i].nrefs > maxrefs ? b.item[i].nrefs : maxrefs;
        totrefs += b.item[i].nrefs;
    }
    const int nblk = b.item[0].nblk;
    if (nblk <= 0 || maxrefs == 0 || search1_skip()) return;
    if (search1_split((size_t)nblk * totrefs, false))
        VP8_LAUNCH(k_search1_b<true>, dim3((nblk + S1Map<true>::BLOCKS_PER_WG - 1) / S1Map<true>::BLOCKS_PER_WG, maxrefs, n), dim3(256), 0, s, b);
    else if (search1_pre_lds() && search1_ref_loop())
        VP8_LAUNCH(k_search1_plr_b, dim3(s1_fill_grid(nblk), 1, n), dim3(256), 0, s, b);
    else if (search1_pre_lds())
        VP8_LAUNCH(k_search1_pl_b, dim3((nblk + S1Map<false>::BLOCKS_PER_WG - 1) / S1Map<false>::BLOCKS_PER_WG, maxrefs, n), dim3(256), 0, s, b);
    else
        VP8_LAUNCH(k_search1_b<false>, dim3((nblk + S1Map<false>::BLOCKS_PER_WG - 1) / S1Map<false>::BLOCKS_PER_WG, maxrefs, n), dim3(256), 0, s, b);
}

__global__ __launch_bounds__(256) void k_weight_tap(const int32_t *d, int n, int32_t *out) {
    const int i = blockIdx.x * 256 + threadIdx.x;
    if (i >= n) return;
    uint32_t cc[4], pp[4];
#pragma unroll
    for (int c = 0; c < 4; ++c) {
        cc[c] = pp[c] = 0;
#pragma unroll
        for (int r = 0; r < 4; ++r) {
            const int v = d[i * 16 + 4 * r + c];
            const uint32_t cb = (uint32_t)(v > 0 ? v : 0) ^ 0x80u, pb = (uint32_t)(v > 0 ? 0 : -v) ^ 0x80u;
            cc[c] |= cb << (8 * r);
            pp[c] |= pb << (8 * r);
        }
    }
    int pre[16];
#pragma unroll
    for (int c = 0; c < 4; ++c) weight_pre_column(cc[c], pre + 4 * c);
    out[i] = weight_cols_pre(pre, pp);
}
void launch_weight_tap(hipStream_t s, const int32_t *d, int n, int32_t *out) {
    hipLaunchKernelGGL(k_weight_tap, dim3((n + 255) / 256), dim3(256), 0, s, d, n, out);
}
__global__ __attribute__((amdgpu_waves_per_eu(8, 8))) __launch_bounds__(256) void k_weight_tap_mfma(const int32_t *d, int n, int32_t *out) {
    const int i0 = blockIdx.x * 256 + threadIdx.x, i = i0 < n ? i0 : n - 1;
    uint32_t cc[4];
    v4i pp;
#pragma unroll
    for (int c = 0; c < 4; ++c) {
        uint32_t cw = 0, pw = 0;
#pragma unroll
        for (int r = 0; r < 4; ++r) {
            const int v = d[i * 16 + 4 * r + c];
            const uint32_t cb = (uint32_t)(v > 0 ? v : 0) ^ 0x80u, pb = (uint32_t)(v > 0 ? 0 : -v) ^ 0x80u;
            cw |= cb << (8 * r);
            pw |= pb << (8 * r);
        }
        cc[c] = cw;
        pp[c] = (int)pw;
    }
    int pre[16];
    weight_pre_block(cc, pre);
    v16i c16;
#pragma unroll
    for (int k = 0; k < 16; ++k) c16[k] = pre[k];
    const int w = weight_mfma(metric_a((int)threadIdx.x), c16, pp);
    if (i0 < n) out[i0] = w;
}
void launch_weight_tap_mfma(hipStream_t s, const int32_t *d, int n, int32_t *out) {
    hipLaunchKernelGGL(k_weight_tap_mfma, dim3((n + 255) / 256), dim3(256), 0, s, d, n, out);
}
__global__ __attribute__((amdgpu_waves_per_eu(8, 8))) __launch_bounds__(256) void k_weight_tap_mfma_rows(const int32_t *d, int n, int32_t *out) {
    const int i0 = blockIdx.x * 256 + threadIdx.x, i = i0 < n ? i0 : n - 1;
    uint32_t cc[4] = {0, 0, 0, 0};
    v4i pp = {0, 0, 0, 0};
#pragma unroll
    for (int r = 0; r < 4; ++r) {
        uint32_t pw = 0;
#pragma unroll
        for (int c = 0; c < 4; ++c) {
            const int v = d[i * 16 + 4 * r + c];
            const uint32_t cb = (uint32_t)(v > 0 ? v : 0) ^ 0x80u, pb = (uint32_t)(v > 0 ? 0 : -v) ^ 0x80u;
            cc[c] |= cb << (8 * r);
            pw |= pb << (8 * c);
        }
        pp[r] = (int)pw;
    }
    int pre[16];
    weight_pre_block(cc, pre);
    v16i c16;
#pragma unroll
    for (int k = 0; k < 16; ++k) c16[k] = pre[k];
    const int w = weight_mfma(metric_a_rows((int)threadIdx.x), c16, pp);
    if (i0 < n) out[i0] = w;
}
void launch_weight_tap_mfma_rows(hipStream_t s, const int32_t *d, int n, int32_t *out) {
    hipLaunchKernelGGL(k_weight_tap_mfma_rows, dim3((n + 255) / 256), dim3(256), 0, s, d, n, out);
}

}
```

Before: 76.19 million.

## Micro-optimize subpel predict, DCT, quant divide, pyramid and pack kernels

Several unrelated micro-optimizations land together. The reciprocal divide becomes a signed mulhi with a sign correction, and the q==1 special case now applies only to DC. Subpel prediction keeps a signed bias through the filter passes with a single final XOR, and the forward DCT drops the pre-scale by 8 using adjusted constants. Zigzag packing now feeds a packed SAD-style nonzero count, reconstruction uses saturating pack instructions, addressing moves to 32-bit offsets, the pyramid kernel uses dot4 and sad instructions, and frame packing is restructured into row-based 16-byte copies. Each piece aims to cut ALU instruction count or improve memory access width, but the arithmetic changes carry some risk of bit-exactness drift.

```diff
diff --git a/vp8oclenc_amd/csrc/kernels_mb.hip b/vp8oclenc_amd/csrc/kernels_mb.hip
--- a/vp8oclenc_amd/csrc/kernels_mb.hip
+++ b/vp8oclenc_amd/csrc/kernels_mb.hip
@@ -6,21 +6,17 @@
 namespace vp8 {
 
 
-struct TDiv { uint32_t M8; bool one; };
 struct Recip24 { uint32_t m8[512]; };
 static constexpr Recip24 make_recip24() {
     Recip24 t{};
-    for (uint32_t q = 0; q < 512; ++q) t.m8[q] = q < 2 ? 0u : (((1u << 24) / q + 1u) << 8);
+    for (uint32_t q = 0; q < 512; ++q) t.m8[q] = q < 3 ? 0u : (((1u << 24) / q + 1u) << 8);
     return t;
 }
 static __device__ __constant__ const Recip24 k_recip24 = make_recip24();
-__device__ __forceinline__ TDiv tdiv_make(int q) { return TDiv{k_recip24.m8[q & 511], q == 1}; }
-__device__ __forceinline__ int tdiv(int x, const TDiv &d) {
-    const int s = x >> 31;
-    const uint32_t n = (uint32_t)((x ^ s) - s);
-    const uint32_t r = d.one ? n : __umulhi(n, d.M8);
-    return ((int)r ^ s) - s;
-}
+typedef int TDiv;
+__device__ __forceinline__ TDiv tdiv_make(int q) { return (int)k_recip24.m8[q & 511]; }
+__device__ __forceinline__ int tdiv(int x, TDiv m8) { return __mulhi(x, m8) - (x >> 31); }
+__device__ __forceinline__ int mb_dc_div(int x, int q) { return q == 1 ? x : tdiv(x, tdiv_make(q)); }
 
 constexpr uint32_t pk8t(int a, int b, int c, int d) {
     return (uint32_t)(a & 255) | ((uint32_t)(b & 255) << 8) | ((uint32_t)(c & 255) << 16) | ((uint32_t)(d & 255) << 24);
@@ -32,16 +28,25 @@
     P6(0, 0, 0, 0, 0, 0),       P6(0, -6, 123, 12, -1, 0), P6(2, -11, 108, 36, -8, 1), P6(0, -9, 93, 50, -6, 0),
     P6(3, -16, 77, 77, -16, 3), P6(0, -6, 50, 93, -9, 0),  P6(1, -8, 36, 108, -11, 2), P6(0, -1, 12, 123, -6, 0)};
 constexpr int KB6 = 128 * 128 + 64;
+constexpr int KR6 = 64;
 __device__ __forceinline__ int d4k(uint32_t a, uint32_t b, int c) { return __builtin_amdgcn_sdot4((int)a, (int)b, c, true); }
 __device__ __forceinline__ int d4(uint32_t a, uint32_t b, int c) { return __builtin_amdgcn_sdot4((int)a, (int)b, c, false); }
-__device__ __forceinline__ void six_tap4(uint32_t w0, uint32_t w1, uint32_t w2, const uint32_t t[9], int s[4]) {
-    s[0] = d4(w1, t[1], d4k(w0, t[0], KB6));
-    s[1] = d4(w1, t[3], d4k(w0, t[2], KB6));
-    s[2] = d4(w1, t[5], d4k(w0, t[4], KB6));
-    s[3] = d4(w2, t[8], d4(w1, t[7], d4k(w0, t[6], KB6)));
+__device__ __forceinline__ void six_tap4(uint32_t w0, uint32_t w1, uint32_t w2, const uint32_t t[9], int s[4], int k0) {
+    s[0] = d4(w1, t[1], d4k(w0, t[0], k0));
+    s[1] = d4(w1, t[3], d4k(w0, t[2], k0));
+    s[2] = d4(w1, t[5], d4k(w0, t[4], k0));
+    s[3] = d4(w2, t[8], d4(w1, t[7], d4k(w0, t[6], k0)));
+}
+typedef unsigned short mb_us2 __attribute__((ext_vector_type(2)));
+__device__ __forceinline__ uint32_t low_half(unsigned short v) {
+    return __builtin_bit_cast(uint32_t, __builtin_shufflevector(mb_us2{v, 0}, mb_us2{0, 0}, 0, -1));
 }
 __device__ __forceinline__ uint32_t pack_sat4(const int s[4]) {
-    const uint32_t lo = __builtin_amdgcn_ashr_pk_u8_i32(s[0], s[1], 7), hi = __builtin_amdgcn_ashr_pk_u8_i32(s[2], s[3], 7);
+    const uint32_t lo = low_half(__builtin_amdgcn_ashr_pk_i8_i32(s[0], s[1], 7)), hi = low_half(__builtin_amdgcn_ashr_pk_i8_i32(s[2], s[3], 7));
+    return __builtin_amdgcn_perm(hi, lo, 0x05040100u);
+}
+__device__ __forceinline__ uint32_t pack_satu4(const int s[4]) {
+    const uint32_t lo = low_half(__builtin_amdgcn_ashr_pk_u8_i32(s[0], s[1], 0)), hi = low_half(__builtin_amdgcn_ashr_pk_u8_i32(s[2], s[3], 0));
     return __builtin_amdgcn_perm(hi, lo, 0x05040100u);
 }
 template <bool CONFORMANT>
@@ -50,21 +55,23 @@
 #pragma unroll
     for (int i = 0; i < 9; ++i) { tx[i] = K_P6[fx][i]; ty[i] = K_P6[fy][i]; }
     uint32_t Hb[9];
+    const uint8_t *line = rf.p + (ptrdiff_t)(iy - 2) * rf.stride + (ix - 2);
 #pragma unroll
     for (int L = 0; L < 9; ++L) {
-        const uint8_t *p = rf.p + (ptrdiff_t)(iy - 2 + L) * rf.stride + (ix - 2);
+        const uint8_t *p = line + (ptrdiff_t)L * rf.stride;
         const uint32_t w0 = ld_u32(p) ^ 0x80808080u, w1 = ld_u32(p + 4) ^ 0x80808080u, w2 = ld_u32(p + 8) ^ 0x80808080u;
         int sm[4];
-        six_tap4(w0, w1, w2, tx, sm);
         uint32_t h;
         if (L < 6 || CONFORMANT) {
+            six_tap4(w0, w1, w2, tx, sm, KR6);
             h = pack_sat4(sm);
         } else {
+            six_tap4(w0, w1, w2, tx, sm, KB6);
             h = 0;
 #pragma unroll
             for (int c = 0; c < 4; ++c) h |= (uint32_t)(div128(sm[c]) & 0xff) << (8 * c);
-        }
-        h ^= 0x80808080u;
+            h ^= 0x80808080u;
+        }
         Hb[L] = fx == 0 ? __builtin_amdgcn_alignbyte(w1, w0, 2) : h;
     }
     uint32_t ca[4], cb[4], oc[4];
@@ -73,34 +80,45 @@
 #pragma unroll
     for (int c = 0; c < 4; ++c) {
         int sm[4];
-        six_tap4(ca[c], cb[c], Hb[8] >> (8 * c), ty, sm);
+        six_tap4(ca[c], cb[c], Hb[8] >> (8 * c), ty, sm, KR6);
         const uint32_t v = pack_sat4(sm);
-        oc[c] = fy == 0 ? (__builtin_amdgcn_alignbyte(cb[c], ca[c], 2) ^ 0x80808080u) : v;
+        oc[c] = fy == 0 ? __builtin_amdgcn_alignbyte(cb[c], ca[c], 2) : v;
     }
     transpose4x4(oc, out);
-}
-
+#pragma unroll
+    for (int r = 0; r < 4; ++r) out[r] ^= 0x80808080u;
+}
+
+constexpr uint32_t K_ROT4_A = 8868u | (21408u << 16);
+constexpr uint32_t K_ROT4_B = (uint32_t)(-21408 & 0xffff) | (8868u << 16);
 __device__ __forceinline__ void fdct4x4(const int in[16], int out[16]) {
     int L[16];
 #pragma unroll
     for (int c = 0; c < 4; ++c) {
         const int r0 = in[c], r1 = in[4 + c], r2 = in[8 + c], r3 = in[12 + c];
-        const int a1 = (r0 + r3) * 8, d1 = (r0 - r3) * 8, b1 = (r1 + r2) * 8, c1 = (r1 - r2) * 8;
+        const int a1 = r0 + r3, d1 = r0 - r3, b1 = r1 + r2, c1 = r1 - r2;
         L[c] = a1 + b1;
         L[8 + c] = a1 - b1;
         const uint32_t xy = pk16(c1, d1);
-        L[4 + c] = dot2(xy, K_ROT_A, 14500) >> 12;
-        L[12 + c] = dot2(xy, K_ROT_B, 7500) >> 12;
+        L[4 + c] = dot2(xy, K_ROT4_A, 7250) >> 11;
+        L[12 + c] = dot2(xy, K_ROT4_B, 3750) >> 11;
     }
 #pragma unroll
     for (int i = 0; i < 4; ++i) {
         const int e0 = L[4 * i], e1 = L[4 * i + 1], e2 = L[4 * i + 2], e3 = L[4 * i + 3];
         const int a1 = e0 + e3, d1 = e0 - e3, b1 = e1 + e2, c1 = e1 - e2;
-        out[4 * i] = (a1 + b1 + 7) >> 4;
-        out[4 * i + 2] = (a1 - b1 + 7) >> 4;
         const uint32_t xy = pk16(c1, d1);
-        out[4 * i + 1] = (dot2(xy, K_ROT_A, 12000) >> 16) + (d1 != 0);
-        out[4 * i + 3] = dot2(xy, K_ROT_B, 51000) >> 16;
+        if (i & 1) {
+            out[4 * i] = (a1 + b1 + 7) >> 4;
+            out[4 * i + 2] = (a1 - b1 + 7) >> 4;
+            out[4 * i + 1] = (dot2(xy, K_ROT_A, 12000) >> 16) + (d1 != 0);
+            out[4 * i + 3] = dot2(xy, K_ROT_B, 51000) >> 16;
+        } else {
+            out[4 * i] = (a1 + b1) >> 1;
+            out[4 * i + 2] = (a1 - b1) >> 1;
+            out[4 * i + 1] = (dot2(xy, K_ROT_A, 1500) >> 13) + (d1 != 0);
+            out[4 * i + 3] = dot2(xy, K_ROT_B, 6375) >> 13;
+        }
     }
 }
 
@@ -134,7 +152,7 @@
     const int s1 = i >= 2 ? -1 : 1, s2 = (i == 1 || i == 2) ? -1 : 1, s3 = (i & 1) ? -1 : 1;
     return v0 + __mul24(s1, v1) + __mul24(s2, v2) + __mul24(s3, v3);
 }
-__device__ __forceinline__ int wht_roundtrip_lane(int x, int lane, int dc_q, int ac_q, const TDiv &ddc, const TDiv &dac, int &q) {
+__device__ __forceinline__ int wht_roundtrip_lane(int x, int lane, int dc_q, int ac_q, TDiv ddc, TDiv dac, int &q) {
     const int L = lane & 15, r = L >> 2, c = L & 3;
     const int base = (int)(threadIdx.x & 32u) * 4;
     const int col = base + 4 * c, row = base + 4 * (L & 12);
@@ -155,16 +173,23 @@
     return t[k];
 }
 __device__ __forceinline__ int inv_zigzag_rt(int k) { return (int)((0xfea9db83c7426510ull >> (4 * k)) & 15); }
-__device__ __forceinline__ void store_zigzag(int16_t *dst, const int L[16]) {
+__device__ __forceinline__ void pack_zigzag(const int L[16], uint32_t w[8]) {
     int z[16];
 #pragma unroll
     for (int k = 0; k < 16; ++k) z[inv_zigzag(k)] = L[k];
-    uint32_t w[8];
-#pragma unroll
-    for (int k = 0; k < 8; ++k) w[k] = (uint32_t)(uint16_t)z[2 * k] | ((uint32_t)(uint16_t)z[2 * k + 1] << 16);
+#pragma unroll
+    for (int k = 0; k < 8; ++k) w[k] = pk16(z[2 * k], z[2 * k + 1]);
+}
+__device__ __forceinline__ void store_zigzag(int16_t *dst, const uint32_t w[8]) {
     uint4 *d4 = reinterpret_cast<uint4 *>(dst);
     d4[0] = make_uint4(w[0], w[1], w[2], w[3]);
     d4[1] = make_uint4(w[4], w[5], w[6], w[7]);
+}
+__device__ __forceinline__ int nz_zigzag(const uint32_t w[8], uint32_t dc_mask, int acc) {
+    uint32_t s = abs_acc(as_s16x2(w[0] & dc_mask), (uint32_t)acc);
+#pragma unroll
+    for (int k = 1; k < 8; ++k) s = abs_acc(as_s16x2(w[k]), s);
+    return (int)s;
 }
 
 struct MBPlanes { uint8_t *y, *u, *v; };
@@ -253,6 +278,7 @@
     uint8_t *const rpu = ref == 0 ? a.ref0.u : (ref == 1 ? a.ref1.u : a.ref2.u);
     uint8_t *const rpv = ref == 0 ? a.ref0.v : (ref == 1 ? a.ref1.v : a.ref2.v);
     const int pstride = plane == 0 ? a.ystride : a.cstride, pw = plane == 0 ? a.yw : a.cw, ph = plane == 0 ? a.yh : a.ch;
+    const uint32_t pix0 = (uint32_t)(posy * pstride + posx);
     const Plane cp{plane == 0 ? a.cur.y : (plane == 1 ? a.cur.u : a.cur.v), pstride, pw, ph};
     const Plane rc{plane == 0 ? a.recon.y : (plane == 1 ? a.recon.u : a.recon.v), pstride, pw, ph};
     const Plane rp{plane == 0 ? rpy : (plane == 1 ? rpu : rpv), pstride, pw, ph};
@@ -270,7 +296,7 @@
         predict4x4<CONFORMANT>(rp, ix, iy, dx, dy, predw);
 #pragma unroll
         for (int r = 0; r < 4; ++r) {
-            const uint32_t cw = *reinterpret_cast<const uint32_t *>(cp.p + (ptrdiff_t)(posy + r) * cp.stride + posx);
+            const uint32_t cw = *reinterpret_cast<const uint32_t *>(cp.p + (size_t)(pix0 + (uint32_t)(r * pstride)));
             *reinterpret_cast<uint32_t *>(&s_t[g].cur[tile_off + (by * 4 + r) * msz + bx * 4]) = cw;
         }
     }
@@ -307,6 +333,7 @@
     float ssim = -2.0f;
     int seg_final = a.o_seg[mb];
     int nz_blk = 0;
+    const uint32_t dc_mask = (plane == 0 && parts == 0) ? 0xffff0000u : 0xffffffffu;
     bool any_pass = false;
 
     for (int seg = 3; seg >= 0; --seg) {
@@ -335,8 +362,8 @@
                 for (int c = 0; c < 4; ++c) res[4 * r + c] = byte_of(cw, c) - byte_of(predw[r], c);
             }
             fdct4x4(res, coef);
-            const TDiv ddc = tdiv_make(dc_q), dac = tdiv_make(ac_q);
-            coef[0] = tdiv(coef[0], ddc);
+            const TDiv dac = tdiv_make(ac_q);
+            coef[0] = mb_dc_div(coef[0], dc_q);
 #pragma unroll
             for (int k = 1; k < 16; ++k) coef[k] = tdiv(coef[k], dac);
         }
@@ -353,22 +380,23 @@
             }
         }
         if (blk) {
-            if (live) store_zigzag(a.o_coeffs + ((size_t)mb * 25 + lane) * 16, coef);
-#pragma unroll
-            for (int k = 1; k < 16; ++k) nz_blk += iabs((int16_t)coef[k]);
-            if (plane != 0 || parts != 0) nz_blk += iabs((int16_t)coef[0]);
+            uint32_t zw[8];
+            pack_zigzag(coef, zw);
+            if (live) store_zigzag(a.o_coeffs + ((size_t)mb * 25 + lane) * 16, zw);
+            nz_blk = nz_zigzag(zw, dc_mask, nz_blk);
             int L[16];
             L[0] = __mul24((int16_t)coef[0], dc_q);
 #pragma unroll
-            for (int k = 1; k < 16; ++k) L[k] = __mul24((int16_t)coef[k], ac_q);
+            for (int k = 1; k < 16; ++k) L[k] = __mul24(coef[k], ac_q);
             idct4x4(L);
 #pragma unroll
             for (int r = 0; r < 4; ++r) {
-                uint32_t w = 0;
-#pragma unroll
-                for (int c = 0; c < 4; ++c) w |= (uint32_t)sat8(L[4 * r + c] + byte_of(predw[r], c)) << (8 * c);
+                int px[4];
+#pragma unroll
+                for (int c = 0; c < 4; ++c) px[c] = L[4 * r + c] + byte_of(predw[r], c);
+                const uint32_t w = pack_satu4(px);
                 *reinterpret_cast<uint32_t *>(&s_t[g].rec[tile_off + (by * 4 + r) * msz + bx * 4]) = w;
-                if (live) *reinterpret_cast<uint32_t *>(rc.p + (ptrdiff_t)(posy + r) * rc.stride + posx) = w;
+                if (live) *reinterpret_cast<uint32_t *>(rc.p + (size_t)(pix0 + (uint32_t)(r * pstride))) = w;
             }
         }
         }
@@ -456,7 +484,7 @@
     }
     return acc;
 }
-__device__ __forceinline__ int wht_roundtrip_row(int x, int L, int base_bytes, int dc_q, int ac_q, const TDiv &ddc, const TDiv &dac, int &q) {
+__device__ __forceinline__ int wht_roundtrip_row(int x, int L, int base_bytes, int dc_q, int ac_q, TDiv ddc, TDiv dac, int &q) {
     const int r = L >> 2, c = L & 3;
     const int col = base_bytes + 4 * c, row = base_bytes + 4 * (L & 12);
     auto gather_col = [&](int v, int i) { return had4(__builtin_amdgcn_ds_bpermute(col, v), __builtin_amdgcn_ds_bpermute(col + 16, v),
@@ -517,6 +545,7 @@
     uint8_t *const rpu = ref == 0 ? a.ref0.u : (ref == 1 ? a.ref1.u : a.ref2.u);
     uint8_t *const rpv = ref == 0 ? a.ref0.v : (ref == 1 ? a.ref1.v : a.ref2.v);
     const int pstride = luma ? a.ystride : a.cstride, pw = luma ? a.yw : a.cw, ph = luma ? a.yh : a.ch;
+    const uint32_t pix0 = (uint32_t)(posy * pstride + posx);
     const Plane cp{plane == 0 ? a.cur.y : (plane == 1 ? a.cur.u : a.cur.v), pstride, pw, ph};
     const Plane rc{plane == 0 ? a.recon.y : (plane == 1 ? a.recon.u : a.recon.v), pstride, pw, ph};
     const Plane rp{plane == 0 ? rpy : (plane == 1 ? rpu : rpv), pstride, pw, ph};
@@ -535,7 +564,7 @@
         predict4x4<CONFORMANT>(rp, ix, iy, dx, dy, predw);
 #pragma unroll
         for (int r = 0; r < 4; ++r) {
-            const uint32_t cw = *reinterpret_cast<const uint32_t *>(cp.p + (ptrdiff_t)(posy + r) * cp.stride + posx);
+            const uint32_t cw = *reinterpret_cast<const uint32_t *>(cp.p + (size_t)(pix0 + (uint32_t)(r * pstride)));
             *reinterpret_cast<uint32_t *>(&T.cur[tile_off + (by * 4 + r) * msz + bx * 4]) = cw;
         }
     }
@@ -578,6 +607,7 @@
     float ssim = -2.0f;
     int seg_final = a.o_seg[mb];
     int nz_y = 0, nz_c = 0;
+    const uint32_t dc_mask = (luma && parts == 0) ? 0xffff0000u : 0xffffffffu;
     bool any_pass = false;
     for (int seg = 3, round = 0; seg >= 0; --seg, ++round) {
         const bool act = !(ssim > a.ssim_target);
@@ -603,8 +633,8 @@
                     for (int c = 0; c < 4; ++c) res[4 * r + c] = byte_of(cw, c) - byte_of(predw[r], c);
                 }
                 fdct4x4(res, coef);
-                const TDiv ddc = tdiv_make(dc_q), dac = tdiv_make(ac_q);
-                coef[0] = tdiv(coef[0], ddc);
+                const TDiv dac = tdiv_make(ac_q);
+                coef[0] = mb_dc_div(coef[0], dc_q);
 #pragma unroll
                 for (int k = 1; k < 16; ++k) coef[k] = tdiv(coef[k], dac);
             }
@@ -619,22 +649,23 @@
                 nz_blk += iabs((int16_t)q24);
             }
             {
-                if (live) store_zigzag(a.o_coeffs + ((size_t)mb * 25 + blkidx) * 16, coef);
-#pragma unroll
-                for (int k = 1; k < 16; ++k) nz_blk += iabs((int16_t)coef[k]);
-                if (!luma || parts != 0) nz_blk += iabs((int16_t)coef[0]);
+                uint32_t zw[8];
+                pack_zigzag(coef, zw);
+                if (live) store_zigzag(a.o_coeffs + ((size_t)mb * 25 + blkidx) * 16, zw);
+                nz_blk = nz_zigzag(zw, dc_mask, nz_blk);
                 int L[16];
                 L[0] = __mul24((int16_t)coef[0], dc_q);
 #pragma unroll
-                for (int k = 1; k < 16; ++k) L[k] = __mul24((int16_t)coef[k], ac_q);
+                for (int k = 1; k < 16; ++k) L[k] = __mul24(coef[k], ac_q);
                 idct4x4(L);
 #pragma unroll
                 for (int r = 0; r < 4; ++r) {
-                    uint32_t wd = 0;
-#pragma unroll
-                    for (int c = 0; c < 4; ++c) wd |= (uint32_t)sat8(L[4 * r + c] + byte_of(predw[r], c)) << (8 * c);
+                    int px[4];
+#pragma unroll
+                    for (int c = 0; c < 4; ++c) px[c] = L[4 * r + c] + byte_of(predw[r], c);
+                    const uint32_t wd = pack_satu4(px);
                     *reinterpret_cast<uint32_t *>(&T.rec[tile_off + (by * 4 + r) * msz + bx * 4]) = wd;
-                    if (live) *reinterpret_cast<uint32_t *>(rc.p + (ptrdiff_t)(posy + r) * rc.stride + posx) = wd;
+                    if (live) *reinterpret_cast<uint32_t *>(rc.p + (size_t)(pix0 + (uint32_t)(r * pstride))) = wd;
                 }
             }
             if (luma) nz_y = row_sum(nz_blk);
diff --git a/vp8oclenc_amd/csrc/kernels_me.hip b/vp8oclenc_amd/csrc/kernels_me.hip
--- a/vp8oclenc_amd/csrc/kernels_me.hip
+++ b/vp8oclenc_amd/csrc/kernels_me.hip
@@ -35,8 +35,8 @@
 static int border_jobs(const Frame &f) { return (f.Y[0].h + 2 * EXT) + 2 * (f.U.h + 2 * EXT); }
 
 __global__ __launch_bounds__(256) void k_pyramid(PyrArgs a) {
-    __shared__ uint8_t s2[16][16];
-    __shared__ uint8_t s3[8][8];
+    __shared__ __attribute__((aligned(4))) uint8_t s2[16][16];
+    __shared__ __attribute__((aligned(4))) uint8_t s3[8][8];
     const Frame &f = a.f[blockIdx.z];
     const int t = threadIdx.x, tx = t & 15, ty = t >> 4;
     const Plane &P0 = f.Y[0];
@@ -52,47 +52,56 @@
         else if (job < ny + 2 * nc) border_row(f.V, job - ny - nc - EXT, t & 63);
         return;
     }
-    const int sx = imin(bx * 64 + 4 * tx, P0.w - 4), sy0 = by * 64 + 4 * ty;
+    static_assert(PAD >= 4, "a clamped row is read from its first byte");
+    const int x0 = bx * 64 + 4 * tx, sy0 = by * 64 + 4 * ty;
+    const bool in = x0 < P0.w && sy0 < P0.h;
+    const uint32_t last = (uint32_t)((P0.h - 1) * P0.stride + (P0.w - 4));
+    const uint32_t o0 = __umul24((uint32_t)imin(sy0, P0.h - 1), (uint32_t)P0.stride) + (uint32_t)imin(x0, P0.w - 4);
+    uint32_t lim = in ? 0xffffffffu : last;
+    asm("" : "+v"(lim));
     uint32_t r[4];
 #pragma unroll
-    for (int k = 0; k < 4; ++k)
-        r[k] = *reinterpret_cast<const uint32_t *>(P0.p + (ptrdiff_t)imin(sy0 + k, P0.h - 1) * P0.stride + sx);
-    int l1[2][2];
+    for (int k = 0; k < 4; ++k) {
+        const uint32_t o = o0 + (uint32_t)(k * P0.stride);
+        r[k] = *reinterpret_cast<const uint32_t *>(P0.p + (size_t)(k == 0 ? o : __builtin_elementwise_min(o, lim)));
+    }
+    uint32_t l1[2][2];
 #pragma unroll
     for (int j = 0; j < 2; ++j)
 #pragma unroll
-        for (int i = 0; i < 2; ++i)
-            l1[j][i] = (byte_of(r[2 * j], 2 * i) + byte_of(r[2 * j], 2 * i + 1) + byte_of(r[2 * j + 1], 2 * i) +
-                        byte_of(r[2 * j + 1], 2 * i + 1) + 2) >> 2;
-    const Plane &P1 = f.Y[1];
-    const int x1 = bx * 32 + 2 * tx, y1 = by * 32 + 2 * ty;
-    if (x1 < P1.w) {
+        for (int i = 0; i < 2; ++i) {
+            const uint32_t pick = i == 0 ? 0x00000101u : 0x01010000u;
+            l1[j][i] = __builtin_amdgcn_udot4(r[2 * j], pick, __builtin_amdgcn_udot4(r[2 * j + 1], pick, 2u, false), false) >> 2;
+        }
+    const uint32_t l2 = (l1[0][0] + l1[0][1] + l1[1][0] + l1[1][1] + 2) >> 2;
+    if (in) {
+        const Plane &P1 = f.Y[1];
+        const uint32_t o1 = __umul24((uint32_t)(by * 32 + 2 * ty), (uint32_t)P1.stride) + (uint32_t)(bx * 32 + 2 * tx);
 #pragma unroll
         for (int j = 0; j < 2; ++j)
-            if (y1 + j < P1.h)
-                *reinterpret_cast<uint16_t *>(P1.p + (ptrdiff_t)(y1 + j) * P1.stride + x1) = (uint16_t)(l1[j][0] | (l1[j][1] << 8));
-    }
-    const int l2 = (l1[0][0] + l1[0][1] + l1[1][0] + l1[1][1] + 2) >> 2;
-    const Plane &P2 = f.Y[2];
-    const int x2 = bx * 16 + tx, y2 = by * 16 + ty;
-    if (x2 < P2.w && y2 < P2.h) P2.p[(ptrdiff_t)y2 * P2.stride + x2] = (uint8_t)l2;
+            *reinterpret_cast<uint16_t *>(P1.p + (size_t)(o1 + (uint32_t)(j * P1.stride))) = (uint16_t)(l1[j][0] | (l1[j][1] << 8));
+        const Plane &P2 = f.Y[2];
+        P2.p[(size_t)(__umul24((uint32_t)(by * 16 + ty), (uint32_t)P2.stride) + (uint32_t)(bx * 16 + tx))] = (uint8_t)l2;
+    }
     s2[ty][tx] = (uint8_t)l2;
     __syncthreads();
     if (t < 64) {
         const int ux = t & 7, uy = t >> 3;
-        const int l3 = (s2[2 * uy][2 * ux] + s2[2 * uy][2 * ux + 1] + s2[2 * uy + 1][2 * ux] + s2[2 * uy + 1][2 * ux + 1] + 2) >> 2;
+        const uint32_t a0 = *reinterpret_cast<const uint16_t *>(&s2[2 * uy][2 * ux]), a1 = *reinterpret_cast<const uint16_t *>(&s2[2 * uy + 1][2 * ux]);
+        const uint32_t l3 = __builtin_amdgcn_sad_u8(a0, 0u, __builtin_amdgcn_sad_u8(a1, 0u, 2u)) >> 2;
         const Plane &P3 = f.Y[3];
         const int x3 = bx * 8 + ux, y3 = by * 8 + uy;
-        if (x3 < P3.w && y3 < P3.h) P3.p[(ptrdiff_t)y3 * P3.stride + x3] = (uint8_t)l3;
+        if (x3 < P3.w && y3 < P3.h) P3.p[(size_t)(__umul24((uint32_t)y3, (uint32_t)P3.stride) + (uint32_t)x3)] = (uint8_t)l3;
         s3[uy][ux] = (uint8_t)l3;
     }
     __syncthreads();
     if (t < 16) {
         const int ux = t & 3, uy = t >> 2;
-        const int l4 = (s3[2 * uy][2 * ux] + s3[2 * uy][2 * ux + 1] + s3[2 * uy + 1][2 * ux] + s3[2 * uy + 1][2 * ux + 1] + 2) >> 2;
+        const uint32_t a0 = *reinterpret_cast<const uint16_t *>(&s3[2 * uy][2 * ux]), a1 = *reinterpret_cast<const uint16_t *>(&s3[2 * uy + 1][2 * ux]);
+        const uint32_t l4 = __builtin_amdgcn_sad_u8(a0, 0u, __builtin_amdgcn_sad_u8(a1, 0u, 2u)) >> 2;
         const Plane &P4 = f.Y[4];
         const int x4 = bx * 4 + ux, y4 = by * 4 + uy;
-        if (x4 < P4.w && y4 < P4.h) P4.p[(ptrdiff_t)y4 * P4.stride + x4] = (uint8_t)l4;
+        if (x4 < P4.w && y4 < P4.h) P4.p[(size_t)(__umul24((uint32_t)y4, (uint32_t)P4.stride) + (uint32_t)x4)] = (uint8_t)l4;
     }
 }
 
@@ -117,40 +126,52 @@
 }
 
 struct PackItem { Plane py, pu, pv; const uint8_t *sy, *su, *sv; int sw, sh, ssy, ssc; };
-__device__ __forceinline__ void pack_body(const PackItem &a, int per) {
-    const Plane &py = a.py, &pu = a.pu, &pv = a.pv;
-    const uint8_t *sy = a.sy, *su = a.su, *sv = a.sv;
-    const int ny = (py.w >> 3) * py.h, nc = (pu.w >> 3) * pu.h;
-    for (int k = 0; k < per; ++k) {
-        int i = ((int)blockIdx.x * per + k) * 256 + (int)threadIdx.x;
-        const Plane *pl = &py;
-        const uint8_t *src = sy;
-        int sw = a.sw, sh = a.sh, ss = a.ssy;
-        if (i >= ny) {
-            i -= ny;
-            pl = &pu;
-            src = su;
-            sw >>= 1; sh >>= 1; ss = a.ssc;
-            if (i >= nc) { i -= nc; pl = &pv; src = sv; }
-            if (i >= nc) return;
-        }
-        const int upr = pl->w >> 3;
-        const int y = i / upr, x = (i % upr) * 8;
+struct PackGrid { int rows_y, wg_y, wg_c; };
+__device__ __forceinline__ void pack_body(const PackItem &a, const PackGrid &g) {
+    int wg = (int)blockIdx.x;
+    const int pi = wg < g.wg_y ? 0 : (wg < g.wg_y + g.wg_c ? 1 : 2);
+    wg -= pi == 0 ? 0 : (pi == 1 ? g.wg_y : g.wg_y + g.wg_c);
+    uint8_t *const dp = pi == 0 ? a.py.p : (pi == 1 ? a.pu.p : a.pv.p);
+    const uint8_t *const src = pi == 0 ? a.sy : (pi == 1 ? a.su : a.sv);
+    const int dstride = pi == 0 ? a.py.stride : a.pu.stride, dw = pi == 0 ? a.py.w : a.pu.w, dh = pi == 0 ? a.py.h : a.pu.h;
+    const int sw = pi == 0 ? a.sw : a.sw >> 1, sh = pi == 0 ? a.sh : a.sh >> 1, ss = pi == 0 ? a.ssy : a.ssc;
+    const int rows = pi == 0 ? g.rows_y : 2 * g.rows_y;
+    const int wave = __builtin_amdgcn_readfirstlane((int)(threadIdx.x >> 6)), lane = (int)(threadIdx.x & 63);
+    const int y_end = imin((wg + 1) * rows, dh);
+    const bool aligned = ((ss | (int)(reinterpret_cast<uintptr_t>(src) & 7)) & 7) == 0;
+    for (int y = wg * rows + wave; y < y_end; y += 4) {
         const uint8_t *row = src + (size_t)(y < sh ? y : sh - 1) * ss;
-        uint2 v;
-        if (x + 8 <= sw && ((ss | (int)(reinterpret_cast<uintptr_t>(src) & 7)) & 7) == 0) {
-            v = *reinterpret_cast<const uint2 *>(row + x);
-        } else {
-            uint32_t w[2] = {0, 0};
-#pragma unroll
-            for (int j = 0; j < 8; ++j) w[j >> 2] |= (uint32_t)row[x + j < sw ? x + j : sw - 1] << (8 * (j & 3));
-            v = make_uint2(w[0], w[1]);
-        }
-        *reinterpret_cast<uint2 *>(pl->p + (ptrdiff_t)y * pl->stride + x) = v;
-    }
-}
-
-__global__ __launch_bounds__(256) void k_pack_b(BatchOf<PackItem> b, int per) { pack_body(b.item[blockIdx.z], per); }
+        uint8_t *drow = dp + (ptrdiff_t)y * dstride;
+        for (int x = lane * 16; x + 16 <= dw; x += 1024) {
+            uint4 v;
+            if (x + 16 <= sw && aligned) {
+                const uint2 v0 = *reinterpret_cast<const uint2 *>(row + (uint32_t)x), v1 = *reinterpret_cast<const uint2 *>(row + (uint32_t)x + 8);
+                v = make_uint4(v0.x, v0.y, v1.x, v1.y);
+            } else {
+                uint32_t w[4] = {0, 0, 0, 0};
+#pragma unroll
+                for (int j = 0; j < 16; ++j) w[j >> 2] |= (uint32_t)row[x + j < sw ? x + j : sw - 1] << (8 * (j & 3));
+                v = make_uint4(w[0], w[1], w[2], w[3]);
+            }
+            *reinterpret_cast<uint4 *>(drow + (uint32_t)x) = v;
+        }
+        if ((dw & 8) && lane == ((dw >> 4) & 63)) {
+            const int x = dw & ~15;
+            uint2 v;
+            if (x + 8 <= sw && aligned) {
+                v = *reinterpret_cast<const uint2 *>(row + (uint32_t)x);
+            } else {
+                uint32_t w[2] = {0, 0};
+#pragma unroll
+                for (int j = 0; j < 8; ++j) w[j >> 2] |= (uint32_t)row[x + j < sw ? x + j : sw - 1] << (8 * (j & 3));
+                v = make_uint2(w[0], w[1]);
+            }
+            *reinterpret_cast<uint2 *>(drow + (uint32_t)x) = v;
+        }
+    }
+}
+
+__global__ __launch_bounds__(256) void k_pack_b(BatchOf<PackItem> b, PackGrid g) { pack_body(b.item[blockIdx.z], g); }
 static int pack_units_per_thread() {
     static const int per = [] { const char *e = getenv("VP8HIP_PACK_UNITS"); const int v = e ? atoi(e) : 16; return v < 1 ? 1 : (v > 64 ? 64 : v); }();
     return per;
@@ -166,9 +187,12 @@
     b.n = n;
     for (int i = 0; i < n; ++i) b.item[i] = pack_item(*items[i].f, items[i].y, items[i].u, items[i].v, sw, sh, ssy, ssc);
     const Frame &f = *items[0].f;
-    const int units = (f.Y[0].w >> 3) * f.Y[0].h + 2 * ((f.U.w >> 3) * f.U.h);
-    const int per = pack_units_per_thread();
-    VP8_LAUNCH(k_pack_b, dim3((units + 256 * per - 1) / (256 * per), 1, n), dim3(256), 0, s, b, per);
+    PackGrid g;
+    g.rows_y = pack_units_per_thread() * 2048 / f.Y[0].w;
+    if (g.rows_y < 1) g.rows_y = 1;
+    g.wg_y = (f.Y[0].h + g.rows_y - 1) / g.rows_y;
+    g.wg_c = (f.U.h + 2 * g.rows_y - 1) / (2 * g.rows_y);
+    VP8_LAUNCH(k_pack_b, dim3(g.wg_y + 2 * g.wg_c, 1, n), dim3(256), 0, s, b, g);
 }
 
 struct Search1Args {
```

Result: faster. 77.16 million, median of 6 (+1.3%).
